# alibaba-damo-academy/Inferix

Hardware: AMD Instinct MI355X
Metric: latent_frames_per_sec (higher is better)
Workload: dtype bf16; 1 GPU; Self-Forcing 480p bf16 (Wan2.1-T2V-1.3B causal DiT, 30 layers), block_size=3, 21 latent frames = 7 blocks x (4 denoise + 1 context) generator forwards, KV prefix 4680..32760 keys in the KV manager's cache (identity page map; page-table form: `streaming_steady`); `value` counts the generator calls (SURVEY 8d), the per-block VAE decode of config 2 is measured beside it under --full (`per_block_decod; batch=1, parallelism=single, layers=30, pair_forwards=True, pair_mode=streams

## Files before the change

include/inferix_hip.h:

```cpp
#ifndef INFERIX_HIP_H
#define INFERIX_HIP_H

#include <stdint.h>

#ifdef __cplusplus
extern "C" {
#endif

#define IFX_OK 0
#define IFX_EINVAL (-1)
#define IFX_ELAUNCH (-2)
#define IFX_EUNSUP (-3)

typedef uint16_t ifx_bf16;

#define IFX_ABI_MINOR 7
int ifx_version(void);
const char* ifx_last_error(void);
const char* ifx_arch(void);
int ifx_set_option(const char* key, int32_t value);
int ifx_get_option(const char* key, int32_t* value);
int32_t ifx_device_error(int32_t clear);

typedef struct {
  ifx_bf16* k;
  ifx_bf16* v;
  const int32_t* page_table;
  int32_t page_size;
  int32_t num_slots;
  int32_t kv_heads;
  int32_t head_dim;
  int32_t seg_split;
  int32_t seg_delta;
} ifx_kv_view;

int ifx_attn_fwd_paged(const ifx_bf16* q, ifx_bf16* out, float* lse, const ifx_kv_view* kv,
                       int32_t q_rows, int32_t heads, int32_t kv_start, int32_t kv_len, float scale,
                       void* stream);

int32_t ifx_attn_split_plan(int32_t q_rows, int32_t heads, int32_t kv_start, int32_t kv_len,
                            int64_t* workspace_bytes);
int ifx_attn_fwd_paged_split(const ifx_bf16* q, ifx_bf16* out, float* lse, const ifx_kv_view* kv,
                             int32_t q_rows, int32_t heads, int32_t kv_start, int32_t kv_len, float scale,
                             int32_t num_splits, void* workspace, int64_t workspace_bytes, void* stream);

int ifx_attn_fwd_paged_ld(const ifx_bf16* q, int32_t ldq, ifx_bf16* out, int32_t ldo, float* lse, const ifx_kv_view* kv,
                          int32_t q_rows, int32_t heads, int32_t kv_start, int32_t kv_len, float scale, int32_t num_splits,
                          void* workspace, int64_t workspace_bytes, void* stream);

int ifx_attn_fwd_dedup(const ifx_bf16* q, ifx_bf16* out, const ifx_kv_view* kv, int32_t q_rows, int32_t heads, int32_t kv_len,
                       int32_t last_key_multiplicity, float scale, void* stream);

int ifx_attn_fwd_ranges(const ifx_bf16* q, int32_t ldq, ifx_bf16* out, int32_t ldo, const ifx_kv_view* kv, int32_t q_rows,
                        int32_t heads, int32_t n_ranges, const int32_t* q_ranges, const int32_t* k_ranges, float scale,
                        void* stream);

int ifx_attn_fwd_partial(const ifx_bf16* q, const ifx_kv_view* kv, int32_t q_rows, int32_t heads, int32_t kv_start,
                         int32_t kv_len, float scale, int32_t num_splits, void* workspace, int64_t workspace_bytes,
                         int32_t slot_base, int32_t slot_cap, int32_t* slots_used, void* stream);
int ifx_attn_merge_partials(const void* workspace, int32_t slot_cap, int32_t slots_used, ifx_bf16* out, float* lse,
                            int32_t q_rows, int32_t heads, void* stream);

int ifx_lse_merge(ifx_bf16* out_a, float* lse_a, const ifx_bf16* out_b, const float* lse_b,
                  int32_t rows, int32_t heads, void* stream);

typedef struct {
  const double* freqs;
  int32_t max_pos;
  int32_t start_frame;
  int32_t height, width;
  int32_t hw_offset;
  int32_t hw_local;
  float q_scale;
  int32_t flags;
} ifx_rope_grid;

int ifx_rmsnorm_rope_kv_append(const ifx_bf16* qkv, int32_t qkv_row_stride, ifx_bf16* q_out,
                               const ifx_bf16* wq, const ifx_bf16* wk, const ifx_rope_grid* rope,
                               const ifx_kv_view* kv, int32_t local_start, int32_t rows,
                               int32_t dim, float eps, void* stream);

int ifx_rmsnorm(const ifx_bf16* x, int32_t x_row_stride, ifx_bf16* y, int32_t y_row_stride,
                const ifx_bf16* w, int32_t rows, int32_t dim, float eps, void* stream);

enum { IFX_LN_PLAIN = 0, IFX_LN_AFFINE = 1, IFX_LN_MODULATE = 2 };
int ifx_layernorm(const ifx_bf16* x, ifx_bf16* y, int32_t rows, int32_t dim, float eps, int32_t mode,
                  const ifx_bf16* gamma, const ifx_bf16* beta, const ifx_bf16* mod,
                  int32_t mod_slots, int32_t shift_slot, int32_t scale_slot, int32_t rows_per_group,
                  void* stream);

enum { IFX_EPI_BIAS = 0, IFX_EPI_GELU_TANH = 1, IFX_EPI_RESIDUAL = 2, IFX_EPI_GATE_RES = 3, IFX_EPI_GELU_ERF = 4 };
typedef struct {
  int32_t epilogue;
  const ifx_bf16* residual;
  int32_t ld_res;
  const ifx_bf16* mod;
  int32_t mod_slots;
  int32_t gate_slot;
  int32_t rows_per_group;
  ifx_bf16* y2;
  int32_t ldy2;
  int32_t split_col;
} ifx_epilogue;
int ifx_gemm_bf16(const ifx_bf16* x, int32_t ldx, const ifx_bf16* w, const ifx_bf16* bias,
                  ifx_bf16* y, int32_t ldy, int32_t M, int32_t N, int32_t K,
                  const ifx_epilogue* epi, void* stream);

int64_t ifx_gemm_workspace_bytes(int32_t M, int32_t N, int32_t K);
int ifx_gemm_bf16_ws(const ifx_bf16* x, int32_t ldx, const ifx_bf16* w, const ifx_bf16* bias, ifx_bf16* y, int32_t ldy,
                     int32_t M, int32_t N, int32_t K, const ifx_epilogue* epi, void* workspace, int64_t workspace_bytes,
                     void* stream);

enum { IFX_Q_FP8_E4M3 = 0, IFX_Q_INT8 = 1 };
int ifx_quant_per_token(const ifx_bf16* x, int32_t ldx, void* q, int32_t ldq, float* scale, int32_t rows,
                        int32_t K, int32_t format, void* stream);
int ifx_gemm_q8(const void* xq, int32_t ldx, const float* x_scale, const void* wq, const float* w_scale,
                const ifx_bf16* bias, ifx_bf16* y, int32_t ldy, int32_t M, int32_t N, int32_t K, int32_t format,
                const ifx_epilogue* epi, void* stream);
int64_t ifx_gemm_q8_workspace_bytes(int32_t M, int32_t N, int32_t K);
int ifx_gemm_q8_ws(const void* xq, int32_t ldx, const float* x_scale, const void* wq, const float* w_scale, const ifx_bf16* bias,
                   ifx_bf16* y, int32_t ldy, int32_t M, int32_t N, int32_t K, int32_t format, const ifx_epilogue* epi,
                   void* workspace, int64_t workspace_bytes, void* stream);
int ifx_layernorm_quant(const ifx_bf16* x, void* q, int32_t ldq, float* scale, int32_t rows, int32_t dim, float eps,
                        int32_t mode, const ifx_bf16* gamma, const ifx_bf16* beta, const ifx_bf16* mod, int32_t mod_slots,
                        int32_t shift_slot, int32_t scale_slot, int32_t rows_per_group, int32_t format, void* stream);

int ifx_gemm_q8_quant_out(const void* xq, int32_t ldx, const float* x_scale, const void* wq, const float* w_scale,
                          const ifx_bf16* bias, void* yq, int32_t ldyq, int32_t M, int32_t N, int32_t K, int32_t format,
                          const ifx_epilogue* epi, const float* out_divisor, int32_t via_bf16, void* stream);
int ifx_layernorm_quant_static(const ifx_bf16* x, void* q, int32_t ldq, const float* divisors, int32_t n_out, int32_t rows,
                               int32_t dim, float eps, int32_t mode, const ifx_bf16* gamma, const ifx_bf16* beta,
                               int32_t via_bf16, void* stream);

int ifx_quant_static(const ifx_bf16* x, int32_t ldx, void* q, int32_t ldq, const float* divisor, int32_t divisor_len,
                     float* row_scale, int32_t rows, int32_t K, int32_t format, int32_t via_bf16, void* stream);
int ifx_quant_per_tensor(const ifx_bf16* x, int32_t ldx, void* q, int32_t ldq, float* row_scale, void* amax_workspace,
                         int32_t rows, int32_t K, int32_t format, void* stream);

int ifx_kv_roll(const ifx_kv_view* kv, int32_t sink_tokens, int32_t evicted, int32_t rolled,
                ifx_bf16* scratch, void* stream);

int ifx_kv_scatter_shards(const ifx_bf16* gathered, int32_t world, int32_t frames, int32_t hw_local,
                          int32_t frame_tokens, int32_t local_start, const ifx_kv_view* kv, void* stream);

#define IFX_MAX_PEERS 8
#define IFX_PEER_HANDLE_BYTES 64
typedef struct {
  int32_t count;
  ifx_bf16* k[IFX_MAX_PEERS];
  ifx_bf16* v[IFX_MAX_PEERS];
} ifx_peer_caches;
typedef struct {
  int32_t count;
  int32_t* flags[IFX_MAX_PEERS];
} ifx_peer_flags;
int ifx_peer_alloc(int64_t bytes, int32_t fine_grained, void** ptr);
int ifx_peer_free(void* ptr);
int ifx_peer_export(const void* ptr, uint8_t* handle, int64_t* offset);
int ifx_peer_open(const uint8_t* handle, void** ptr);
int ifx_peer_close(void* ptr);
int ifx_rmsnorm_rope_kv_push(const ifx_bf16* kv_rows, int32_t kv_row_stride, const ifx_bf16* wk, const ifx_rope_grid* rope,
                             const ifx_peer_caches* peers, const ifx_kv_view* geometry, int32_t local_start, int32_t frame_tokens,
                             int32_t slot_hw_local, int32_t slot_hw_offset, int32_t rows, int32_t dim, float eps, void* stream);
int ifx_peer_signal(const ifx_peer_flags* peers, int32_t index, int32_t value, void* stream);
int ifx_peer_wait(const int32_t* flags, int32_t count, int32_t value, int32_t timeout_ms, int32_t* status, void* stream);

typedef struct {
  const ifx_bf16* x;
  int64_t in_frame_stride;
  const int32_t* in_slots;
  int32_t hs, ws, cin, upsample;
  const ifx_bf16* w;
  const ifx_bf16* bias;
  int32_t kt, ks;
  ifx_bf16* y;
  int64_t out_frame_stride;
  const int32_t* out_slots;
  int32_t cout, t_out;
  const ifx_bf16* residual;
  const void* zero_page;
  int32_t in_planar;
} ifx_conv3d_desc;
int ifx_conv3d_cl(const ifx_conv3d_desc* desc, void* stream);

#define IFX_NORM_SILU 1
#define IFX_NORM_OUT_PLANAR 2
int ifx_rmsnorm_cl(const ifx_bf16* x, const ifx_bf16* gamma, ifx_bf16* y, int64_t out_frame_stride,
                   const int32_t* out_slots, int32_t frames, int32_t frame_pixels, int32_t channels,
                   int32_t flags, void* stream);

int ifx_softmax_rows(const ifx_bf16* scores, ifx_bf16* probs, int32_t rows, int32_t cols, int32_t ld, float scale,
                     void* stream);

int ifx_t5_attention(const ifx_bf16* q, int32_t ldq, const ifx_bf16* k, int32_t ldk, const ifx_bf16* v, int32_t ldv,
                     ifx_bf16* out, int32_t ldo, const ifx_bf16* rel_bias, const int32_t* seq_lens, int32_t batch,
                     int32_t seq_len_padded, int32_t heads, void* stream);

int ifx_t5_gated_gelu(const ifx_bf16* gate_fc1, ifx_bf16* h, int32_t rows, int32_t ffn, void* stream);

typedef struct {
  const ifx_bf16* in;
  int32_t ld_in, rows, layout, q_heads, kv_heads, head_dim;
  const float* rope;
  const float *qn_w, *qn_b, *kn_w, *kn_b;
  const ifx_bf16 *xn_w, *xn_b;
  float eps;
  int32_t layernorm_1p;
  ifx_bf16* q_out;
  int32_t ld_q;
  ifx_bf16* qx_out;
  int32_t ld_qx;
  ifx_bf16* k_out;
  ifx_bf16* v_out;
  int32_t ld_kv, kv_head_stride;
  int32_t row0, split, row1;
  float q_scale;
  int32_t rope_half;
  int32_t q_group;
  int64_t q_group_stride;
} ifx_magi_head_prep_desc;
int ifx_magi_head_prep(const ifx_magi_head_prep_desc* desc, void* stream);

int ifx_magi_gate_norm_residual(const ifx_bf16* x, int32_t ldx, const ifx_bf16* residual, int32_t ld_res,
                                const int32_t* condition_map, const ifx_bf16* gate, int32_t ld_gate, const float* norm_w,
                                const float* norm_b, int32_t layernorm_1p, ifx_bf16* y, int32_t ldy, int32_t rows, int32_t dim,
                                float eps, void* stream);

enum { IFX_ACT_SILU = 0, IFX_ACT_TANH = 1 };
int ifx_act_rows(const ifx_bf16* x, ifx_bf16* y, int64_t n, int32_t mode, void* stream);
int ifx_kv_split_rows(const ifx_bf16* kv, ifx_bf16* k_cache, ifx_bf16* v_cache, int32_t rows, int32_t heads, int32_t row0,
                      int32_t split, int32_t row1, void* stream);

#ifdef __cplusplus
}
#endif
#endif
```

inferix_amd/_hip.py:

```python
from __future__ import annotations

import ctypes as C
import os
from typing import Optional

import torch

_HERE = os.path.dirname(os.path.abspath(__file__))
LIB_PATH = os.environ.get("IFX_HIP_LIB", os.path.join(_HERE, "libinferix_hip.so"))

IFX_LN_PLAIN, IFX_LN_AFFINE, IFX_LN_MODULATE = 0, 1, 2
IFX_EPI_BIAS, IFX_EPI_GELU_TANH, IFX_EPI_RESIDUAL, IFX_EPI_GATE_RES, IFX_EPI_GELU_ERF = 0, 1, 2, 3, 4
IFX_ACT_SILU, IFX_ACT_TANH = 0, 1
IFX_Q_FP8_E4M3, IFX_Q_INT8 = 0, 1


class HipLibraryMissing(RuntimeError):
    pass


class HipKernelError(RuntimeError):
    pass


class KvView(C.Structure):
    _fields_ = [("k", C.c_void_p), ("v", C.c_void_p), ("page_table", C.c_void_p),
                ("page_size", C.c_int32), ("num_slots", C.c_int32), ("kv_heads", C.c_int32),
                ("head_dim", C.c_int32), ("seg_split", C.c_int32), ("seg_delta", C.c_int32)]


class RopeGrid(C.Structure):
    _fields_ = [("freqs", C.c_void_p), ("max_pos", C.c_int32), ("start_frame", C.c_int32),
                ("height", C.c_int32), ("width", C.c_int32), ("hw_offset", C.c_int32),
                ("hw_local", C.c_int32), ("q_scale", C.c_float), ("flags", C.c_int32)]


class Conv3dDesc(C.Structure):
    _fields_ = [("x", C.c_void_p), ("in_frame_stride", C.c_int64), ("in_slots", C.POINTER(C.c_int32)),
                ("hs", C.c_int32), ("ws", C.c_int32), ("cin", C.c_int32), ("upsample", C.c_int32),
                ("w", C.c_void_p), ("bias", C.c_void_p), ("kt", C.c_int32), ("ks", C.c_int32),
                ("y", C.c_void_p), ("out_frame_stride", C.c_int64), ("out_slots", C.POINTER(C.c_int32)),
                ("cout", C.c_int32), ("t_out", C.c_int32), ("residual", C.c_void_p), ("zero_page", C.c_void_p),
                ("in_planar", C.c_int32)]


class Epilogue(C.Structure):
    _fields_ = [("epilogue", C.c_int32), ("residual", C.c_void_p), ("ld_res", C.c_int32),
                ("mod", C.c_void_p), ("mod_slots", C.c_int32), ("gate_slot", C.c_int32),
                ("rows_per_group", C.c_int32), ("y2", C.c_void_p), ("ldy2", C.c_int32), ("split_col", C.c_int32)]


class MagiHeadPrepDesc(C.Structure):
    _fields_ = [("inp", C.c_void_p), ("ld_in", C.c_int32), ("rows", C.c_int32), ("layout", C.c_int32),
                ("q_heads", C.c_int32), ("kv_heads", C.c_int32), ("head_dim", C.c_int32), ("rope", C.c_void_p),
                ("qn_w", C.c_void_p), ("qn_b", C.c_void_p), ("kn_w", C.c_void_p), ("kn_b", C.c_void_p),
                ("xn_w", C.c_void_p), ("xn_b", C.c_void_p), ("eps", C.c_float), ("layernorm_1p", C.c_int32),
                ("q_out", C.c_void_p), ("ld_q", C.c_int32), ("qx_out", C.c_void_p), ("ld_qx", C.c_int32),
                ("k_out", C.c_void_p), ("v_out", C.c_void_p), ("ld_kv", C.c_int32), ("kv_head_stride", C.c_int32),
                ("row0", C.c_int32), ("split", C.c_int32), ("row1", C.c_int32), ("q_scale", C.c_float), ("rope_half", C.c_int32),
                ("q_group", C.c_int32), ("q_group_stride", C.c_int64)]


IFX_MAX_PEERS, IFX_PEER_HANDLE_BYTES = 8, 64


class PeerCaches(C.Structure):
    _fields_ = [("count", C.c_int32), ("k", C.c_void_p * IFX_MAX_PEERS), ("v", C.c_void_p * IFX_MAX_PEERS)]


class PeerFlags(C.Structure):
    _fields_ = [("count", C.c_int32), ("flags", C.c_void_p * IFX_MAX_PEERS)]


_vp, _i32, _f32 = C.c_void_p, C.c_int32, C.c_float
SIGNATURES = {
    "ifx_version": (C.c_int, []),
    "ifx_last_error": (C.c_char_p, []),
    "ifx_arch": (C.c_char_p, []),
    "ifx_set_option": (C.c_int, [C.c_char_p, _i32]),
    "ifx_get_option": (C.c_int, [C.c_char_p, C.POINTER(_i32)]),
    "ifx_device_error": (_i32, [_i32]),
    "ifx_attn_fwd_paged": (C.c_int, [_vp, _vp, _vp, C.POINTER(KvView), _i32, _i32, _i32, _i32, _f32, _vp]),
    "ifx_attn_split_plan": (_i32, [_i32, _i32, _i32, _i32, C.POINTER(C.c_int64)]),
    "ifx_attn_fwd_paged_split": (C.c_int, [_vp, _vp, _vp, C.POINTER(KvView), _i32, _i32, _i32, _i32, _f32, _i32, _vp,
                                           C.c_int64, _vp]),
    "ifx_conv3d_cl": (C.c_int, [C.POINTER(Conv3dDesc), _vp]),
    "ifx_rmsnorm_cl": (C.c_int, [_vp, _vp, _vp, C.c_int64, C.POINTER(_i32), _i32, _i32, _i32, _i32, _vp]),
    "ifx_softmax_rows": (C.c_int, [_vp, _vp, _i32, _i32, _i32, _f32, _vp]),
    "ifx_t5_attention": (C.c_int, [_vp, _i32, _vp, _i32, _vp, _i32, _vp, _i32, _vp, _vp, _i32, _i32, _i32, _vp]),
    "ifx_t5_gated_gelu": (C.c_int, [_vp, _vp, _i32, _i32, _vp]),
    "ifx_kv_scatter_shards": (C.c_int, [_vp, _i32, _i32, _i32, _i32, _i32, C.POINTER(KvView), _vp]),
    "ifx_peer_alloc": (C.c_int, [C.c_int64, _i32, C.POINTER(C.c_void_p)]),
    "ifx_peer_free": (C.c_int, [_vp]),
    "ifx_peer_export": (C.c_int, [_vp, C.c_char_p, C.POINTER(C.c_int64)]),
    "ifx_peer_open": (C.c_int, [C.c_char_p, C.POINTER(C.c_void_p)]),
    "ifx_peer_close": (C.c_int, [_vp]),
    "ifx_rmsnorm_rope_kv_push": (C.c_int, [_vp, _i32, _vp, C.POINTER(RopeGrid), C.POINTER(PeerCaches), C.POINTER(KvView), _i32, _i32,
                                           _i32, _i32, _i32, _i32, _f32, _vp]),
    "ifx_peer_signal": (C.c_int, [C.POINTER(PeerFlags), _i32, _i32, _vp]),
    "ifx_peer_wait": (C.c_int, [_vp, _i32, _i32, _i32, _vp, _vp]),
    "ifx_attn_fwd_partial": (C.c_int, [_vp, C.POINTER(KvView), _i32, _i32, _i32, _i32, _f32, _i32, _vp, C.c_int64, _i32,
                                       _i32, C.POINTER(_i32), _vp]),
    "ifx_attn_merge_partials": (C.c_int, [_vp, _i32, _i32, _vp, _vp, _i32, _i32, _vp]),
    "ifx_lse_merge": (C.c_int, [_vp, _vp, _vp, _vp, _i32, _i32, _vp]),
    "ifx_rmsnorm_rope_kv_append": (C.c_int, [_vp, _i32, _vp, _vp, _vp, C.POINTER(RopeGrid), C.POINTER(KvView),
                                             _i32, _i32, _i32, _f32, _vp]),
    "ifx_rmsnorm": (C.c_int, [_vp, _i32, _vp, _i32, _vp, _i32, _i32, _f32, _vp]),
    "ifx_layernorm": (C.c_int, [_vp, _vp, _i32, _i32, _f32, _i32, _vp, _vp, _vp, _i32, _i32, _i32, _i32, _vp]),
    "ifx_gemm_bf16": (C.c_int, [_vp, _i32, _vp, _vp, _vp, _i32, _i32, _i32, _i32, C.POINTER(Epilogue), _vp]),
    "ifx_kv_roll": (C.c_int, [C.POINTER(KvView), _i32, _i32, _i32, _vp, _vp]),
    "ifx_quant_per_token": (C.c_int, [_vp, _i32, _vp, _i32, _vp, _i32, _i32, _i32, _vp]),
    "ifx_layernorm_quant": (C.c_int, [_vp, _vp, _i32, _vp, _i32, _i32, _f32, _i32, _vp, _vp, _vp, _i32, _i32, _i32, _i32, _i32, _vp]),
    "ifx_gemm_q8": (C.c_int, [_vp, _i32, _vp, _vp, _vp, _vp, _vp, _i32, _i32, _i32, _i32, _i32, C.POINTER(Epilogue), _vp]),
    "ifx_gemm_q8_ws": (C.c_int, [_vp, _i32, _vp, _vp, _vp, _vp, _vp, _i32, _i32, _i32, _i32, _i32, C.POINTER(Epilogue), _vp, C.c_int64, _vp]),
    "ifx_gemm_q8_workspace_bytes": (C.c_int64, [_i32, _i32, _i32]),
    "ifx_attn_fwd_paged_ld": (C.c_int, [_vp, _i32, _vp, _i32, _vp, C.POINTER(KvView), _i32, _i32, _i32, _i32, _f32, _i32, _vp,
                                        C.c_int64, _vp]),
    "ifx_gemm_q8_quant_out": (C.c_int, [_vp, _i32, _vp, _vp, _vp, _vp, _vp, _i32, _i32, _i32, _i32, _i32, C.POINTER(Epilogue), _vp, _i32, _vp]),
    "ifx_layernorm_quant_static": (C.c_int, [_vp, _vp, _i32, _vp, _i32, _i32, _i32, _f32, _i32, _vp, _vp, _i32, _vp]),
    "ifx_quant_static": (C.c_int, [_vp, _i32, _vp, _i32, _vp, _i32, _vp, _i32, _i32, _i32, _i32, _vp]),
    "ifx_quant_per_tensor": (C.c_int, [_vp, _i32, _vp, _i32, _vp, _vp, _i32, _i32, _i32, _vp]),
    "ifx_magi_head_prep": (C.c_int, [C.POINTER(MagiHeadPrepDesc), _vp]),
    "ifx_magi_gate_norm_residual": (C.c_int, [_vp, _i32, _vp, _i32, _vp, _vp, _i32, _vp, _vp, _i32, _vp, _i32, _i32, _i32, _f32,
                                              _vp]),
    "ifx_act_rows": (C.c_int, [_vp, _vp, C.c_int64, _i32, _vp]),
    "ifx_kv_split_rows": (C.c_int, [_vp, _vp, _vp, _i32, _i32, _i32, _i32, _i32, _vp]),
    "ifx_attn_fwd_dedup": (C.c_int, [_vp, _vp, C.POINTER(KvView), _i32, _i32, _i32, _i32, _f32, _vp]),
    "ifx_attn_fwd_ranges": (C.c_int, [_vp, _i32, _vp, _i32, C.POINTER(KvView), _i32, _i32, _i32, C.POINTER(_i32), C.POINTER(_i32), _f32, _vp]),
    "ifx_gemm_workspace_bytes": (C.c_int64, [_i32, _i32, _i32]),
    "ifx_gemm_bf16_ws": (C.c_int, [_vp, _i32, _vp, _vp, _vp, _i32, _i32, _i32, _i32, C.POINTER(Epilogue), _vp, C.c_int64, _vp]),
}

_lib: Optional[C.CDLL] = None
ABI_MINOR = 7


def load() -> C.CDLL:
    global _lib
    if _lib is not None:
        return _lib
    if not os.path.exists(LIB_PATH):
        raise HipLibraryMissing(
            f"{LIB_PATH} not found: build it with `python -c 'import __graft_entry__ as g; g.build()'` "
            "(hipcc --offload-arch=gfx950).  inferix_amd has no CPU or eager fallback.")
    lib = C.CDLL(LIB_PATH)
    for name, (res, args) in SIGNATURES.items():
        fn = getattr(lib, name)
        fn.restype = res
        fn.argtypes = args
    got = (lib.ifx_version() >> 8) & 255
    if got != ABI_MINOR:
        raise HipLibraryMissing(f"{LIB_PATH} has ABI minor {got}, these bindings are for {ABI_MINOR} (include/inferix_hip.h "
                                "IFX_ABI_MINOR): rebuild with __graft_entry__.build()")
    _lib = lib
    return lib


def check(rc: int, what: str) -> None:
    if rc != 0:
        msg = load().ifx_last_error().decode("utf-8", "replace")
        raise HipKernelError(f"{what} failed (code {rc}): {msg}")


def version() -> str:
    v = load().ifx_version()
    return f"{v >> 16}.{(v >> 8) & 255}.{v & 255}"
```

inferix_amd/csrc/ifx_core.hip:

```cpp
#include <stdarg.h>
#include <stdlib.h>
#include <string.h>

#include "ifx_common.h"

namespace ifx {
static thread_local char g_err[512] = "";

void set_error(const char* fmt, ...) {
  va_list ap;
  va_start(ap, fmt);
  vsnprintf(g_err, sizeof(g_err), fmt, ap);
  va_end(ap);
}

static int g_gemm_variant = -1, g_gemm_pp_variant = -1, g_attn_variant = -1, g_conv_variant = -1, g_spin_timeout_ms = -1, g_spin_fault = 0;
static thread_local int g_gemm_small_split = -1;
static int opt_or_env(int& slot, const char* env, int dflt = 0) {
  if (slot < 0) {
    const char* e = getenv(env);
    slot = e ? atoi(e) : dflt;
  }
  return slot;
}
int gemm_variant() { return opt_or_env(g_gemm_variant, "IFX_GEMM_VARIANT"); }
int gemm_pp_variant() { return opt_or_env(g_gemm_pp_variant, "IFX_GEMM_PP_VARIANT"); }
int attn_variant() { return opt_or_env(g_attn_variant, "IFX_ATTN_VARIANT"); }
int conv_variant() { return opt_or_env(g_conv_variant, "IFX_CONV_VARIANT"); }
static unsigned* g_attn_dbg = nullptr;
static bool g_attn_dbg_on = false;
unsigned* attn_debug_counter() { return g_attn_dbg_on ? g_attn_dbg : nullptr; }
int gemm_small_split() { return opt_or_env(g_gemm_small_split, "IFX_GEMM_SMALL_SPLIT"); }

static unsigned* g_dev_err = nullptr;
unsigned* device_error_word() {
  if (g_dev_err == nullptr) {
    void* p = nullptr;
    if (hipHostMalloc(&p, 64, hipHostMallocMapped | hipHostMallocPortable) == hipSuccess && p != nullptr) {
      memset(p, 0, 64);
      g_dev_err = (unsigned*)p;
    }
  }
  return g_dev_err;
}
long long spin_timeout_ticks() { return (long long)max(1, opt_or_env(g_spin_timeout_ms, "IFX_SPIN_TIMEOUT_MS", 2000)) * 100000LL; }
int spin_fault() { return g_spin_fault; }
static thread_local char g_err_dev[640] = "";

int check_launch(const char* what) {
  hipError_t e = hipGetLastError();
  if (e != hipSuccess) {
    set_error("%s: launch failed: %s", what, hipGetErrorString(e));
    return IFX_ELAUNCH;
  }
  return IFX_OK;
}
}

extern "C" int ifx_version(void) { return (0 << 16) | (IFX_ABI_MINOR << 8) | 0; }
extern "C" int32_t ifx_device_error(int32_t clear) {
  unsigned* w = ifx::g_dev_err;
  if (w == nullptr) return 0;
  const unsigned v = __atomic_load_n(w, __ATOMIC_ACQUIRE);
  if (v != 0 && clear) __atomic_store_n(w, 0u, __ATOMIC_RELEASE);
  return (int32_t)v;
}
extern "C" const char* ifx_last_error(void) {
  const unsigned v = (unsigned)ifx_device_error(1);
  if (v == 0) return ifx::g_err;
  const unsigned kind = v >> 24, detail = v & 0xffffffu;
  snprintf(ifx::g_err_dev, sizeof(ifx::g_err_dev),
           "device: a kernel gave up a wait (%s, flag %u) after the spin budget — the producing workgroup was not resident or did not "
           "finish; the results of that launch are invalid%s%s",
           kind == 1 ? "split-K / stream-K consumer of ifx_gemm_bf16_ws / ifx_gemm_q8_ws" : "unknown waiter", detail,
           ifx::g_err[0] ? "; last host error: " : "", ifx::g_err);
  return ifx::g_err_dev;
}
extern "C" const char* ifx_arch(void) { return "gfx950"; }
extern "C" int ifx_set_option(const char* key, int32_t value) {
  if (key && !strcmp(key, "gemm_variant") && value >= 0 && value <= 29) { ifx::g_gemm_variant = value; return IFX_OK; }
  if (key && !strcmp(key, "gemm_small_split") && (value == 0 || value == 1)) { ifx::g_gemm_small_split = value; return IFX_OK; }
  if (key && !strcmp(key, "attn_variant") && value >= 0 && value <= 7) { ifx::g_attn_variant = value; return IFX_OK; }
  if (key && !strcmp(key, "conv_variant") && value >= 0 && value <= 1) { ifx::g_conv_variant = value; return IFX_OK; }
  if (key && !strcmp(key, "gemm_pp_variant") && value >= 0 && value <= 1) { ifx::g_gemm_pp_variant = value; return IFX_OK; }
  if (key && !strcmp(key, "attn_debug_counters") && (value == 0 || value == 1)) {
    if (value == 1) {
      if (ifx::g_attn_dbg == nullptr && hipMalloc((void**)&ifx::g_attn_dbg, 64) != hipSuccess) {
        ifx::g_attn_dbg = nullptr;
        ifx::set_error("ifx_set_option: attn_debug_counters: hipMalloc failed");
        return IFX_ELAUNCH;
      }
      (void)hipDeviceSynchronize();
      (void)hipMemset(ifx::g_attn_dbg, 0, 64);
    }
    ifx::g_attn_dbg_on = value == 1;
    return IFX_OK;
  }
  if (key && !strcmp(key, "spin_timeout_ms") && value >= 1 && value <= 600000) { ifx::g_spin_timeout_ms = value; return IFX_OK; }
  if (key && !strcmp(key, "spin_fault") && (value == 0 || value == 1)) { ifx::g_spin_fault = value; return IFX_OK; }
  ifx::set_error("ifx_set_option: unknown key or value out of range: %s = %d", key ? key : "(null)", (int)value);
  return IFX_EINVAL;
}
extern "C" int ifx_get_option(const char* key, int32_t* value) {
  if (key == nullptr || value == nullptr) { ifx::set_error("ifx_get_option: null argument"); return IFX_EINVAL; }
  if (!strcmp(key, "gemm_variant")) { *value = ifx::gemm_variant(); return IFX_OK; }
  if (!strcmp(key, "gemm_small_split")) { *value = ifx::gemm_small_split(); return IFX_OK; }
  if (!strcmp(key, "attn_variant")) { *value = ifx::attn_variant(); return IFX_OK; }
  if (!strcmp(key, "conv_variant")) { *value = ifx::conv_variant(); return IFX_OK; }
  if (!strcmp(key, "gemm_pp_variant")) { *value = ifx::gemm_pp_variant(); return IFX_OK; }
  if (!strcmp(key, "attn_debug_counters")) { *value = ifx::g_attn_dbg_on ? 1 : 0; return IFX_OK; }
  if (!strcmp(key, "attn_rescale_count")) {
    unsigned v = 0;
    if (ifx::g_attn_dbg != nullptr) {
      (void)hipDeviceSynchronize();
      (void)hipMemcpy(&v, ifx::g_attn_dbg, sizeof(v), hipMemcpyDeviceToHost);
    }
    *value = (int32_t)(v & 0x7fffffffu);
    return IFX_OK;
  }
  if (!strcmp(key, "spin_timeout_ms")) { *value = (int32_t)(ifx::spin_timeout_ticks() / 100000LL); return IFX_OK; }
  if (!strcmp(key, "spin_fault")) { *value = ifx::spin_fault(); return IFX_OK; }
  ifx::set_error("ifx_get_option: unknown key: %s", key);
  return IFX_EINVAL;
}
```

inferix_amd/csrc/ifx_gemm.hip:

```cpp
#include <stdlib.h>

#include "ifx_gemm_epilogue.h"

namespace ifx {

constexpr int BM = 128, BN = 128, BK = 64;

template <int EPI>
__global__ __launch_bounds__(256, 2) void gemm_bf16_kernel(const unsigned short* __restrict__ x, int ldx,
                                                           const unsigned short* __restrict__ w,
                                                           unsigned short* __restrict__ y, int ldy, int M, int N,
                                                           int K, int tiles_m, int tiles_n, EpiArgs ea) {
  extern __shared__ __attribute__((aligned(16))) unsigned char smem[];
  const int tid = threadIdx.x, lane = tid & 63, wave = tid >> 6;
  const int wm = wave & 1, wn = wave >> 1;
  constexpr int GM = 8;
  const int total = tiles_m * tiles_n, per_xcd = (total + 7) / 8;
  const int t_id = (blockIdx.x & 7) * per_xcd + (blockIdx.x >> 3);
  if ((int)(blockIdx.x >> 3) >= per_xcd || t_id >= total) return;
  const int grp_sz = GM * tiles_n;
  const int first_m = (t_id / grp_sz) * GM;
  const int gm = min(GM, tiles_m - first_m);
  const int rem = t_id % grp_sz;
  const int tile_m = first_m + rem % gm, tile_n = rem / gm;
  const int m_base = tile_m * BM, n_base = tile_n * BN;

  const unsigned short* gx[4];
  const unsigned short* gw[4];
  int lds_off[4];
#pragma unroll
  for (int p = 0; p < 4; ++p) {
    const int q = tid + 256 * p, row = q >> 3, c = q & 7;
    const int mr = min(m_base + row, M - 1), nr = min(n_base + row, N - 1);
    gx[p] = x + (size_t)mr * ldx + c * 8;
    gw[p] = w + (size_t)nr * K + c * 8;
    lds_off[p] = row * 128 + ((c ^ (row & 7)) << 4);
  }
  u32x4 rx[4], rw[4];
  auto gload = [&](int kt) {
#pragma unroll
    for (int p = 0; p < 4; ++p) {
      rx[p] = *reinterpret_cast<const u32x4*>(gx[p] + (size_t)kt * BK);
      rw[p] = *reinterpret_cast<const u32x4*>(gw[p] + (size_t)kt * BK);
    }
  };
  auto lstore = [&](int buf) {
    unsigned char* bx = smem + buf * 32768;
    unsigned char* bw = bx + 16384;
#pragma unroll
    for (int p = 0; p < 4; ++p) {
      *reinterpret_cast<u32x4*>(bx + lds_off[p]) = rx[p];
      *reinterpret_cast<u32x4*>(bw + lds_off[p]) = rw[p];
    }
  };

  f32x4 acc[4][4];
#pragma unroll
  for (int i = 0; i < 4; ++i)
#pragma unroll
    for (int j = 0; j < 4; ++j) acc[i][j] = f32x4{0.f, 0.f, 0.f, 0.f};

  const int KT = K / BK;
  gload(0);
  lstore(0);
  __syncthreads();

  const int fr = lane & 15, fq = lane >> 4;
  for (int kt = 0; kt < KT; ++kt) {
    const int buf = kt & 1;
    if (kt + 1 < KT) gload(kt + 1);
    const unsigned char* bx = smem + buf * 32768;
    const unsigned char* bw = bx + 16384;
#pragma unroll
    for (int ks = 0; ks < 2; ++ks) {
      bf16x8 a[4], b[4];
      const int c = ks * 4 + fq;
#pragma unroll
      for (int i = 0; i < 4; ++i) {
        const int row = wn * 64 + i * 16 + fr;
        a[i] = *reinterpret_cast<const bf16x8*>(bw + row * 128 + ((c ^ (row & 7)) << 4));
      }
#pragma unroll
      for (int j = 0; j < 4; ++j) {
        const int row = wm * 64 + j * 16 + fr;
        b[j] = *reinterpret_cast<const bf16x8*>(bx + row * 128 + ((c ^ (row & 7)) << 4));
      }
#pragma unroll
      for (int i = 0; i < 4; ++i)
#pragma unroll
        for (int j = 0; j < 4; ++j)
          acc[i][j] = __builtin_amdgcn_mfma_f32_16x16x32_bf16(a[i], b[j], acc[i][j], 0, 0, 0);
    }
    if (kt + 1 < KT) lstore(buf ^ 1);
    __syncthreads();
  }

#pragma unroll
  for (int j = 0; j < 4; ++j) {
    const int m = m_base + wm * 64 + j * 16 + fr;
    if (m >= M) continue;
    const unsigned short* gate_row = nullptr;
    if (EPI == IFX_EPI_GATE_RES)
      gate_row = ea.mod + ((size_t)(m / ea.rows_per_group) * ea.mod_slots + ea.gate_slot) * N;
#pragma unroll
    for (int i = 0; i < 4; ++i) {
      const int n = n_base + wn * 64 + i * 16 + fq * 4;
      if (n >= N) continue;
      float v[4] = {acc[i][j][0], acc[i][j][1], acc[i][j][2], acc[i][j][3]};
      if (ea.bias) {
        const u16x4 bv = *reinterpret_cast<const u16x4*>(ea.bias + n);
#pragma unroll
        for (int e = 0; e < 4; ++e) v[e] += bf2f(bv[e]);
      }
      u16x4 vb, rv = {}, gv = {};
#pragma unroll
      for (int e = 0; e < 4; ++e) vb[e] = f2bf(v[e]);
      if (EPI == IFX_EPI_RESIDUAL || EPI == IFX_EPI_GATE_RES)
        rv = *reinterpret_cast<const u16x4*>(ea.residual + (size_t)m * ea.ld_res + n);
      if (EPI == IFX_EPI_GATE_RES) gv = *reinterpret_cast<const u16x4*>(gate_row + n);
      const u16x4 o = epi_combine<EPI, 4>(vb, rv, gv, ea.gelu_erf());
      *reinterpret_cast<u16x4*>(y + (size_t)m * ldy + n) = o;
    }
  }
}

static int pick_pp(int M, int N, int K, int mode, bool have_ws) {
  if (N % 64 != 0 || K % 64 != 0) return 0;
  if (have_ws && gemm_pp_split(N, K) && ((M + 255) / 256) * ((N + 255) / 256) <= 1024 && !(gemm_small_split() && M < 2048)) {
    const int tn = (N + 255) / 256, steps = K / 64 / 2;
    const int i4 = ((M + 255) / 256) * tn * 2, i3 = ((M + 191) / 192) * tn * 2;
    const float t4 = ((i4 + 255) / 256) * (steps * 1.6f + 9.f), t3 = ((i3 + 255) / 256) * (steps * 1.4f + 9.f);
    static int allow3 = -1;
    if (allow3 < 0) {
      const char* e = getenv("IFX_PP_SPLIT_TJ3");
      allow3 = e ? atoi(e) : 1;
    }
    return (allow3 && i3 <= 2048 && t3 < t4 && mode != IFX_EPI_GELU_TANH) ? 3 : 4;
  }
  if (M < 1024) return 0;
  static const float step_us[5] = {0.f, 0.f, 1.2f, 1.4f, 1.6f};
  const float tile_us = (mode == IFX_EPI_GELU_TANH ? 8.f : 3.f);
  int best = 0, best_tiles = 0;
  float best_t = 1e30f;
  for (int tj = 4; tj >= 2; --tj) {
    const int tiles = ((M + 64 * tj - 1) / (64 * tj)) * ((N + 255) / 256);
    const int rounds = (tiles + 255) / 256;
    const float t = rounds * ((K / 64) * step_us[tj] + tile_us);
    if (t < best_t) best_t = t, best = tj, best_tiles = tiles;
  }
  if (M < 2048 && best_tiles < 160) return 0;
  return best;
}

static bool want_w4_splitk(int M, int N, int K) {
  const int tiles = ((M + 255) / 256) * ((N + 255) / 256);
  return K >= 4096 && (K / 64) % 2 == 0 && 2 * tiles <= 256 && 2 * tiles >= 160;
}

static int pick_tile(int M, int N, int K) {
  struct Cand { int tile, bm, bn, slots; float base; };
  static const Cand cands[] = {{3, 256, 256, 256, 1.00f}, {19, 256, 192, 256, 0.99f}, {0, 256, 128, 256, 0.85f}, {1, 128, 128, 512, 0.95f},
                               {4, 128, 64, 512, 0.68f},  {2, 64, 64, 512, 0.50f}};
  const int kt = K / 64;
  const int wgs64 = ((M + 63) / 64) * ((N + 63) / 64);
  if (gemm_small_split()) {
    if (wgs64 <= 256 && kt >= 64 && kt % 2 == 0) return 11;
    if (wgs64 <= 256 && kt >= 16 && kt % 4 == 0) return 10;
  }
  const int wgs12864 = ((M + 127) / 128) * ((N + 63) / 64);
  if (wgs12864 > 256 && wgs12864 <= 768) return 13;
  {
    const int t256 = ((M + 255) / 256) * ((N + 255) / 256), rounds = (t256 + 255) / 256;
    if (K >= 2048 && t256 >= 384 && (float)t256 >= 0.7f * 256.f * rounds) return 17;
  }
  int best = 2;
  float best_score = -1.f;
  for (const Cand& c : cands) {
    const int tm = (M + c.bm - 1) / c.bm, tn = (N + c.bn - 1) / c.bn, wgs = tm * tn;
    const int rounds = (wgs + c.slots - 1) / c.slots;
    const float edge = ((float)M * (float)N) / ((float)(tm * c.bm) * (float)(tn * c.bn));
    if (c.tile == 3 && wgs < c.slots && edge < 0.95f) continue;
    const float score = c.base * edge * (float)wgs / (float)(c.slots * rounds);
    if (score > best_score) best_score = score, best = c.tile;
  }
  return best;
}

}

using namespace ifx;

static bool small_split_takes_tile12(int M, int N, int K) {
  if (!gemm_small_split() || N > 2048 || (K / 64) % 2 != 0 || K < 1024) return false;
  const int wgs128 = ((M + 127) / 128) * ((N + 127) / 128);
  return wgs128 > 128 && wgs128 <= 256;
}

static bool small_split_takes_pp_ks4(int M, int N, int K) {
  if (!gemm_small_split() || M >= 2048 || N > 2048 || N % 64 != 0 || K < 4096 || K % 64 != 0 || (K / 64) % 4 != 0) return false;
  const int items = ((M + 127) / 128) * ((N + 255) / 256) * 4;
  return items > 128 && items <= 256;
}

static int gemm_bf16_impl(const ifx_bf16* x, int32_t ldx, const ifx_bf16* w, const ifx_bf16* bias, ifx_bf16* y,
                          int32_t ldy, int32_t M, int32_t N, int32_t K, const ifx_epilogue* epi, void* stream, void* workspace,
                          int64_t workspace_bytes) {
  IFX_REQUIRE(x && w && y && M >= 0 && N > 0 && K > 0, "ifx_gemm_bf16: null/empty operand");
  IFX_REQUIRE(K % BK == 0, "ifx_gemm_bf16: K (%d) must be a multiple of %d", K, BK);
  IFX_REQUIRE(N % 4 == 0 && ldx % 8 == 0 && ldy % 4 == 0, "ifx_gemm_bf16: N %% 4, ldx %% 8, ldy %% 4 required");
  int mode;
  EpiArgsP ea;
  if (const int rc = resolve_epilogue(epi, bias, "ifx_gemm_bf16", &mode, &ea)) return rc;
  if (M == 0) return IFX_OK;
  const int variant = gemm_variant();
  const bool wide_ok = N % 8 == 0 && ldy % 8 == 0 && (ea.residual == nullptr || ea.ld_res % 8 == 0);
  if (wide_ok && variant == 20 && workspace != nullptr && want_w4_splitk(M, N, K) &&
      workspace_bytes >= (int64_t)gemm_w4_workspace_bytes(M, N, 2))
    return launch_gemm_w4(x, ldx, w, y, ldy, M, N, K, mode, ea, (hipStream_t)stream, 2, workspace);
  if (wide_ok && variant == 26 && N % 64 == 0 && K % 64 == 0 && workspace != nullptr &&
      workspace_bytes >= (int64_t)gemm_pp_stream_k_workspace_bytes() && (long)((M + 127) / 128) * ((N + 255) / 256) * (K / 64) >= 48) {
    if (pp_epilogue_fits(mode, ea, 64))
      return launch_gemm_pp(x, ldx, w, y, ldy, M, N, K, mode, ea, (hipStream_t)stream, 2, workspace, 1);
  }
  if (epi != nullptr && epi->y2 != nullptr) {
    IFX_REQUIRE(mode == IFX_EPI_BIAS && wide_ok && N % 64 == 0 && !((uintptr_t)bias & 7) && (variant == 0 || (variant >= 22 && variant <= 25)),
                "ifx_gemm_bf16: the second destination (y2) needs the bias epilogue, N %% 64 == 0, 8-byte aligned bias and the ping-pong tiles");
    int tj = variant == 0 ? pick_pp(M, N, K, mode, false) : (variant == 22 || variant == 25 ? 4 : variant == 23 ? 3 : 2);
    if (tj == 0) tj = 2;
    ea.y2 = epi->y2, ea.ldy2 = epi->ldy2, ea.split_col = epi->split_col;
    return launch_gemm_pp(x, ldx, w, y, ldy, M, N, K, mode, ea, (hipStream_t)stream, tj, nullptr);
  }
  if (wide_ok && variant >= 27 && variant <= 29) {
    const int ks = 2 << (variant - 27);
    const bool fits = N % 64 == 0 && K % 64 == 0 && (K / 64) % ks == 0 && workspace != nullptr &&
                      workspace_bytes >= (int64_t)gemm_pp_small_workspace_bytes(M, N, ks) &&
                      (long)((M + 127) / 128) * ((N + 255) / 256) * (ks - 1) <= 1024 && pp_epilogue_fits(mode, ea, 64);
    if (fits)
      return launch_gemm_pp(x, ldx, w, y, ldy, M, N, K, mode, ea, (hipStream_t)stream, 2, workspace, 0, 0, ks);
  }
  if (wide_ok && variant == 0 && small_split_takes_pp_ks4(M, N, K) && workspace != nullptr &&
      workspace_bytes >= (int64_t)gemm_pp_small_workspace_bytes(M, N, 4)) {
    if (pp_epilogue_fits(mode, ea, 64))
      return launch_gemm_pp(x, ldx, w, y, ldy, M, N, K, mode, ea, (hipStream_t)stream, 2, workspace, 0, 0, 4);
  }
  if (wide_ok && variant == 0 && small_split_takes_tile12(M, N, K))
    return launch_gemm_lds_dma(12, x, ldx, w, y, ldy, M, N, K, mode, ea, (hipStream_t)stream);
  if (wide_ok && (variant == 0 || (variant >= 22 && variant <= 25))) {
    const bool ws_ok = workspace != nullptr && workspace_bytes >= (int64_t)gemm_pp_workspace_bytes(M, N, K) && variant != 25;
    int tj = variant == 0 ? pick_pp(M, N, K, mode, ws_ok) : (variant == 22 || variant == 25 ? 4 : variant == 23 ? 3 : 2);
    const bool fits = N % 64 == 0 && pp_epilogue_fits(mode, ea, 32 * tj);
    if (tj && (fits || variant != 0))
      return launch_gemm_pp(x, ldx, w, y, ldy, M, N, K, mode, ea, (hipStream_t)stream, tj, ws_ok ? workspace : nullptr);
  }
  if (wide_ok && variant != 1) {
    const int tile = (variant >= 2 && variant != 20 && variant != 26) ? variant - 2 : pick_tile(M, N, K);
    return launch_gemm_lds_dma(tile, x, ldx, w, y, ldy, M, N, K, mode, ea, (hipStream_t)stream);
  }
  const int tiles_m = (M + BM - 1) / BM, tiles_n = (N + BN - 1) / BN;
  const dim3 grid(((tiles_m * tiles_n + 7) / 8) * 8), block(256);
  const size_t lds = 65536;
  hipStream_t s = (hipStream_t)stream;
  const int rc = dispatch_epilogue(mode, "ifx_gemm_bf16", [&](auto epi_c) {
    constexpr int E = decltype(epi_c)::value;
    static bool attr_set = false;
    if (!attr_set) {
      (void)hipFuncSetAttribute((const void*)gemm_bf16_kernel<E>, hipFuncAttributeMaxDynamicSharedMemorySize, (int)lds);
      attr_set = true;
    }
    hipLaunchKernelGGL((gemm_bf16_kernel<E>), grid, block, lds, s, x, ldx, w, y, ldy, M, N, K, tiles_m, tiles_n, ea);
  });
  if (rc != IFX_OK) return rc;
  return check_launch("ifx_gemm_bf16");
}

extern "C" int ifx_gemm_bf16(const ifx_bf16* x, int32_t ldx, const ifx_bf16* w, const ifx_bf16* bias, ifx_bf16* y,
                             int32_t ldy, int32_t M, int32_t N, int32_t K, const ifx_epilogue* epi, void* stream) {
  return gemm_bf16_impl(x, ldx, w, bias, y, ldy, M, N, K, epi, stream, nullptr, 0);
}

extern "C" int64_t ifx_gemm_workspace_bytes(int32_t M, int32_t N, int32_t K) {
  if (M <= 0 || N <= 0 || K <= 0) return 0;
  const int v = gemm_variant();
  if (v == 20) return want_w4_splitk(M, N, K) ? (int64_t)gemm_w4_workspace_bytes(M, N, 2) : 0;
  if (v == 26 && N % 64 == 0 && K % 64 == 0) return (int64_t)gemm_pp_stream_k_workspace_bytes();
  if (v >= 27 && v <= 29) return (N % 64 == 0 && K % 64 == 0 && (K / 64) % (2 << (v - 27)) == 0) ? (int64_t)gemm_pp_small_workspace_bytes(M, N, 2 << (v - 27)) : 0;
  if (v == 0 && small_split_takes_pp_ks4(M, N, K)) return (int64_t)gemm_pp_small_workspace_bytes(M, N, 4);
  if (v == 0 && N % 8 == 0 && small_split_takes_tile12(M, N, K)) return 0;
  if ((v == 0 && N % 64 == 0 && K % 64 == 0 && !(gemm_small_split() && M < 2048)) || v == 22) return (int64_t)gemm_pp_workspace_bytes(M, N, K);
  return 0;
}

extern "C" int ifx_gemm_bf16_ws(const ifx_bf16* x, int32_t ldx, const ifx_bf16* w, const ifx_bf16* bias, ifx_bf16* y,
                                int32_t ldy, int32_t M, int32_t N, int32_t K, const ifx_epilogue* epi, void* workspace,
                                int64_t workspace_bytes, void* stream) {
  return gemm_bf16_impl(x, ldx, w, bias, y, ldy, M, N, K, epi, stream, workspace, workspace_bytes);
}
```

inferix_amd/csrc/ifx_gemm_epilogue.h:

```cpp
#pragma once
#include <type_traits>

#include "ifx_common.h"

namespace ifx {

struct EpiArgs {
  const unsigned short* bias = nullptr;
  const unsigned short* residual = nullptr;
  int ld_res = 0;
  const unsigned short* mod = nullptr;
  int mod_slots = 1, gate_slot = 0, rows_per_group = 1;
  __host__ __device__ bool gelu_erf() const { return gate_slot != 0; }
};

struct EpiArgsQ : EpiArgs {
  const float* sa = nullptr;
  const float* sw = nullptr;
  const float* qdiv = nullptr;
  int q_via_bf16 = 0;
};

struct EpiArgsP : EpiArgsQ {
  unsigned short* y2 = nullptr;
  int ldy2 = 0, split_col = 0;
};

template <int W>
using u16v = unsigned short __attribute__((ext_vector_type(W)));

template <int EPI, int W>
__device__ __forceinline__ u16v<W> epi_combine(const u16v<W> vv, const u16v<W> rv, const u16v<W> gv, const bool erf) {
  u16v<W> o;
  if constexpr (EPI == IFX_EPI_BIAS) {
    o = vv;
  } else if constexpr (EPI == IFX_EPI_GELU_TANH) {
    if (erf) {
#pragma unroll
      for (int e = 0; e < W; ++e) o[e] = f2bf(gelu_erf_f(bf2f(vv[e])));
    } else {
#pragma unroll
      for (int e = 0; e < W; ++e) o[e] = f2bf(gelu_tanh_fast(bf2f(vv[e])));
    }
  } else if constexpr (EPI == IFX_EPI_RESIDUAL) {
#pragma unroll
    for (int e = 0; e < W; ++e) o[e] = f2bf(bf2f(rv[e]) + bf2f(vv[e]));
  } else {
    static_assert(EPI == IFX_EPI_GATE_RES, "epilogue");
#pragma unroll
    for (int e = 0; e < W; ++e) o[e] = f2bf(bf2f(rv[e]) + rbf(bf2f(vv[e]) * bf2f(gv[e])));
  }
  return o;
}

template <int EPI, int W>
__device__ __forceinline__ u16v<W> epi_apply(const u16v<W> vv, int m, int n, int N, const EpiArgs& ea) {
  u16v<W> rv = vv, gv = vv;
  if constexpr (EPI == IFX_EPI_RESIDUAL || EPI == IFX_EPI_GATE_RES)
    rv = *reinterpret_cast<const u16v<W>*>(ea.residual + (size_t)m * ea.ld_res + n);
  if constexpr (EPI == IFX_EPI_GATE_RES)
    gv = *reinterpret_cast<const u16v<W>*>(ea.mod + ((size_t)(m / ea.rows_per_group) * ea.mod_slots + ea.gate_slot) * N + n);
  return epi_combine<EPI, W>(vv, rv, gv, ea.gelu_erf());
}

template <int EPI>
__device__ __forceinline__ void epi_store_row(const u16x8 vv, int m, int n, int N, const EpiArgs& ea, unsigned short* __restrict__ y,
                                              int ldy) {
  *reinterpret_cast<u16x8*>(y + (size_t)m * ldy + n) = epi_apply<EPI, 8>(vv, m, n, N, ea);
}


template <typename F>
static inline int dispatch_epilogue(int mode, const char* what, F&& launch) {
  switch (mode) {
    case IFX_EPI_BIAS: launch(std::integral_constant<int, IFX_EPI_BIAS>{}); return IFX_OK;
    case IFX_EPI_GELU_TANH: launch(std::integral_constant<int, IFX_EPI_GELU_TANH>{}); return IFX_OK;
    case IFX_EPI_RESIDUAL: launch(std::integral_constant<int, IFX_EPI_RESIDUAL>{}); return IFX_OK;
    case IFX_EPI_GATE_RES: launch(std::integral_constant<int, IFX_EPI_GATE_RES>{}); return IFX_OK;
    default: set_error("%s: unknown epilogue %d", what, mode); return IFX_EINVAL;
  }
}

static inline int resolve_epilogue(const ifx_epilogue* epi, const unsigned short* bias, const char* who, int* mode, EpiArgs* ea) {
  *mode = epi ? epi->epilogue : IFX_EPI_BIAS;
  *ea = EpiArgs{};
  ea->bias = bias;
  if (*mode == IFX_EPI_GELU_ERF) {
    *mode = IFX_EPI_GELU_TANH;
    ea->gate_slot = 1;
  }
  if (*mode == IFX_EPI_RESIDUAL || *mode == IFX_EPI_GATE_RES) {
    IFX_REQUIRE(epi->residual && epi->ld_res % 4 == 0, "%s: residual epilogue needs residual/ld_res", who);
    ea->residual = epi->residual;
    ea->ld_res = epi->ld_res;
  }
  if (*mode == IFX_EPI_GATE_RES) {
    IFX_REQUIRE(epi->mod && epi->rows_per_group > 0 && epi->gate_slot >= 0 && epi->gate_slot < epi->mod_slots,
                "%s: gate epilogue needs mod/mod_slots/gate_slot/rows_per_group", who);
    ea->mod = epi->mod;
    ea->mod_slots = epi->mod_slots;
    ea->gate_slot = epi->gate_slot;
    ea->rows_per_group = epi->rows_per_group;
  }
  return IFX_OK;
}

static inline bool pp_epilogue_fits(int mode, const EpiArgs& ea, int min_rows_per_group) {
  const bool res = mode == IFX_EPI_RESIDUAL || mode == IFX_EPI_GATE_RES;
  return !((uintptr_t)ea.bias & 7) && (!res || (!((uintptr_t)ea.residual & 15) && ea.ld_res % 8 == 0)) &&
         (mode != IFX_EPI_GATE_RES || (!((uintptr_t)ea.mod & 15) && ea.rows_per_group >= min_rows_per_group));
}

int launch_gemm_lds_dma(int tile, const unsigned short* x, int ldx, const unsigned short* w, unsigned short* y, int ldy, int M, int N,
                        int K, int mode, const EpiArgs& ea, hipStream_t s);
int launch_gemm_glds(const unsigned short* x, int ldx, const unsigned short* w, unsigned short* y, int ldy, int M, int N, int K,
                     int mode, const EpiArgs& ea, hipStream_t s);
int launch_gemm_w4(const unsigned short* x, int ldx, const unsigned short* w, unsigned short* y, int ldy, int M, int N, int K,
                   int mode, const EpiArgs& ea, hipStream_t s, int splits, void* workspace);
size_t gemm_w4_workspace_bytes(int M, int N, int splits);
int launch_gemm_pp(const unsigned short* x, int ldx, const unsigned short* w, unsigned short* y, int ldy, int M, int N, int K,
                   int mode, const EpiArgsP& ea, hipStream_t s, int tj, void* workspace, int stream_k = 0, int q8_int8 = 0,
                   int force_ks = 0);
size_t gemm_pp_small_workspace_bytes(int M, int N, int ks);
size_t gemm_pp_stream_k_workspace_bytes();
bool gemm_pp_split(int N, int K);
size_t gemm_pp_workspace_bytes(int M, int N, int K);

}
```

inferix_amd/csrc/ifx_gemm_pp.hip:

```cpp
#include <stdlib.h>

#include "ifx_gemm_epilogue.h"

#ifndef IFX_PP_TRACE
#define IFX_PP_TRACE 0
#endif
#ifndef IFX_PP_LAB
#define IFX_PP_LAB IFX_PP_TRACE
#endif


namespace ifx {

namespace gpp {
constexpr int BN = 256, BK = 64;
constexpr int SLOT = 16384, STAGE = 4 * SLOT, SCRATCH = 2 * STAGE;
constexpr int LDS_BYTES = SCRATCH + 32768;
constexpr int X_UP = 0, W_LO = SLOT, W_HI = 2 * SLOT, X_DN = 3 * SLOT;
constexpr int LX_STAGE = 16384, LX_DN = 8192, LW_BASE = 32768, LW_STAGE = 32768;
typedef int v4i __attribute__((ext_vector_type(4)));
typedef int v8i __attribute__((ext_vector_type(8)));
typedef int v16i __attribute__((ext_vector_type(16)));
typedef __attribute__((address_space(3))) void* lds_ptr_t;

__device__ __forceinline__ void dma16(v4i rsrc, unsigned lds, int voff, int soff) {
  asm volatile("s_mov_b32 m0, %0\n\ts_nop 0\n\tbuffer_load_dwordx4 %1, %2, %3 offen lds"
               :
               : "s"(lds), "v"(voff), "s"(rsrc), "s"(soff)
               : "memory");
}
__device__ __forceinline__ v4i make_rsrc(const void* base, unsigned num_bytes) {
  const unsigned long long a = (unsigned long long)base;
  v4i r;
  r[0] = (int)(unsigned)a;
  r[1] = (int)((unsigned)(a >> 32) & 0xffffu);
  r[2] = (int)num_bytes;
  r[3] = 0x00020000;
  return r;
}
template <int N>
__device__ __forceinline__ void wait_vm() {
  asm volatile("s_waitcnt vmcnt(%0)" ::"n"(N) : "memory");
}
template <int N, bool ON>
__device__ __forceinline__ void wait_vm_if() {
  if constexpr (ON) wait_vm<N>();
}
__device__ __forceinline__ void wait_lds() { __builtin_amdgcn_s_waitcnt(0xC07F); }

struct Cursor {
  int i, kt, g, rot, k0, len;
  int kb;
  unsigned stg;
  v4i rs;
};
}

template <int EPI, int TJ, int KS, int Q8 = 0, int LW = 0>
__global__ __launch_bounds__(LW ? 768 : 512, LW ? 3 : 2) void gemm_pp_kernel(const unsigned short* __restrict__ x, int ldx,
                                                         const unsigned short* __restrict__ w, unsigned short* __restrict__ y,
                                                         int ldy, int M, int N, int K, int tiles_m, int total, int per_xcd,
                                                         int wg_per_xcd, EpiArgsP ea, unsigned long long* __restrict__ trace, int dbg,
                                                         float* __restrict__ ws_part, unsigned* __restrict__ ws_flag,
                                                         unsigned* __restrict__ err_word, long long spin_ticks) {
  using namespace gpp;
  static_assert(!LW || (TJ == 2 && KS == 1 && Q8 == 0), "the loader-wave form is the unsplit bf16 128-token tile");
  dbg = IFX_PP_LAB ? dbg : (dbg & 32);
  constexpr int BM = 64 * TJ;
  constexpr int GM = 4;
  constexpr bool RES = EPI == IFX_EPI_RESIDUAL || EPI == IFX_EPI_GATE_RES;
  extern __shared__ __attribute__((aligned(16))) unsigned char smem[];
  const int tid = threadIdx.x, lane = tid & 63;
  const int wave = __builtin_amdgcn_readfirstlane(tid >> 6);
  const int grp = wave >> 2, w4 = wave & 3;
  constexpr int ES = Q8 ? 1 : 2;
  const unsigned char* const xb = reinterpret_cast<const unsigned char*>(x);
  const unsigned char* const wb = reinterpret_cast<const unsigned char*>(w);
  constexpr bool SK = KS == 0;
  constexpr int KSD = KS > 0 ? KS : 1;
  const int S = K * ES / 128;
  const int KT = S / KSD;
  const int tiles_n = total / KSD / tiles_m;

  const int xcd = blockIdx.x & 7, slot_i = blockIdx.x >> 3;
  const int id_first = xcd * per_xcd + slot_i;
  const int id_end = min(xcd * per_xcd + per_xcd, total);
  if (!SK && id_first >= id_end) return;
  const int sk_P = (int)gridDim.x, sk_p = xcd * (sk_P >> 3) + slot_i;
  auto sk_start = [&](int q) __attribute__((always_inline)) { return (int)((long)q * total * S / sk_P); };
  const int sk_u0 = SK ? sk_start(sk_p) : 0, sk_u1 = SK ? sk_start(sk_p + 1) : 0;
  const int sk_t0 = SK ? sk_u0 / S : 0;
  const int n_my = SK ? (sk_u1 - 1) / S - sk_t0 + 1 : (id_end - id_first + wg_per_xcd - 1) / wg_per_xcd;
  const int G = SK ? sk_u1 - sk_u0 : n_my * KT;
  auto item_split = [&](int i) __attribute__((always_inline)) { return KS > 1 ? (id_first + i * wg_per_xcd) % KSD : 0; };
  auto item_tile = [&](int i) __attribute__((always_inline)) { return SK ? sk_t0 + i : (id_first + i * wg_per_xcd) / KSD; };
  auto item_k0 = [&](int i) __attribute__((always_inline)) { return SK ? (i == 0 ? sk_u0 - sk_t0 * S : 0) : item_split(i) * KT; };
  auto item_len = [&](int i) __attribute__((always_inline)) {
    return SK ? min(S, sk_u1 - (sk_t0 + i) * S) - (i == 0 ? sk_u0 - sk_t0 * S : 0) : KT;
  };
  auto item_dumps = [&](int i) __attribute__((always_inline)) { return SK ? (i == 0 && sk_u0 > sk_t0 * S) : (KS > 1 && item_split(i) >= 1); };
  auto item_parts = [&](int i) __attribute__((always_inline)) {
    if (!SK) return KS > 1 ? KS - 1 : 0;
    const int t_end = (sk_t0 + i + 1) * S;
    int n = 0;
    while (sk_p + 1 + n < sk_P && sk_start(sk_p + 1 + n) < t_end) ++n;
    return sk_u1 < t_end ? n : 0;
  };
  auto tile_base = [&](int i, int& m_base, int& n_base) __attribute__((always_inline)) {
    const int t_id = item_tile(i);
    const int grp_sz = GM * tiles_n;
    const int first_m = (t_id / grp_sz) * GM;
    const int gm = min(GM, tiles_m - first_m);
    const int rem = t_id % grp_sz;
    m_base = (first_m + rem % gm) * BM;
    n_base = (rem / gm) * BN;
  };

  const int r8 = lane >> 3, pc = lane & 7;
  const int prow = w4 * 8 + r8;
  const int ld_op = grp == 0 ? K : ldx;
  const int voff = prow * ld_op * ES + ((pc ^ ((prow >> 1) & 7)) << 4);
  const int voff_w = LW ? prow * K * ES + ((pc ^ ((prow >> 1) & 7)) << 4) : 0;
  const int voff_x = LW ? prow * ldx * ES + ((pc ^ ((prow >> 1) & 7)) << 4) : 0;
  const unsigned lds_piece0 = (unsigned)(unsigned long long)(lds_ptr_t)smem + w4 * 1024;
  auto cur_desc = [&](Cursor& c, bool is_w) __attribute__((always_inline)) {
    int mb, nb;
    tile_base(c.i, mb, nb);
    if (dbg & 1) mb = nb = 0;
    c.rot = (!SK && (dbg & 4)) ? ((nb / BN) * 3) % KT : 0;
    c.k0 = item_k0(c.i);
    c.len = item_len(c.i);
    c.kb = c.k0 * 128;
    if (is_w) c.rs = make_rsrc(wb + (size_t)nb * K * ES, (unsigned)min(((long)N - nb) * (long)K * ES, 0xffffffffL));
    else c.rs = make_rsrc(xb + (size_t)mb * ldx * ES, (unsigned)min(((long)M - mb - 1) * (long)ldx * ES + (long)K * ES, 0xffffffffL));
  };
  auto cur_init = [&](Cursor& c, bool is_w) __attribute__((always_inline)) {
    c.i = 0, c.kt = 0, c.g = 0, c.stg = 0;
    cur_desc(c, is_w);
  };
  auto cur_next = [&](Cursor& c, bool is_w) __attribute__((always_inline)) {
    ++c.g;
    if constexpr (LW) c.stg = !is_w ? c.stg ^ LX_STAGE : c.stg == 2 * LW_STAGE ? 0 : c.stg + LW_STAGE;
    else c.stg ^= STAGE;
    c.kb += 128;
    if (++c.kt == c.len) {
      c.kt = 0;
      if (++c.i < n_my) cur_desc(c, is_w);
    }
  };
  auto issue = [&](const Cursor& c, bool is_w, int slot, int row0, int pieces) __attribute__((always_inline)) {
    const int kk = c.kt + c.rot;
    const int kb = IFX_PP_LAB ? ((!SK && kk >= KT ? kk - KT : kk) + c.k0) * 128 : c.kb;
    const unsigned p = lds_piece0 + c.stg + slot;
    if ((dbg & 8) && c.g >= 2) return;
    const int vo = LW ? (is_w ? voff_w : voff_x) : voff;
    const int pitch = LW ? (is_w ? K : ldx) : ld_op;
#pragma unroll
    for (int q = 0; q < 4; ++q)
      if (q < pieces) dma16(c.rs, p + q * 4096, vo, kb + (row0 + q * 32) * pitch * ES);
  };
  const bool opw = grp == 0;
  auto req_w = [&](Cursor& c) __attribute__((always_inline)) {
    if constexpr (!LW) issue(c, opw, W_LO, 0, 4), issue(c, opw, W_HI, 128, 4), cur_next(c, opw);
  };
  auto req_x = [&](Cursor& c, int slot, int row0) __attribute__((always_inline)) {
    if constexpr (!LW) issue(c, opw, slot, row0, TJ), cur_next(c, opw);
  };
  Cursor ca, cb;
  cur_init(ca, opw);
  cur_init(cb, opw);

  constexpr bool MF16 = Q8 == 0;
  const int l31 = lane & 31, hi = lane >> 5, l15 = lane & 15, q4 = lane >> 4;
  int lane_ks[4];
#pragma unroll
  for (int ks = 0; ks < 4; ++ks)
    lane_ks[ks] = MF16 ? l15 * 128 + ((((4 * ks + q4) & 7) ^ ((l15 >> 1) & 7)) << 4)
                       : l31 * 128 + (((2 * ks + hi) ^ ((l31 >> 1) & 7)) << 4);
  const int w_frag_off = (w4 >> 1) * SLOT + (w4 & 1) * 8192 + W_LO;
  const int x_frag_off = grp == 0 ? X_UP : X_DN;
  bf16x8 fx[4][TJ], fw[4][2], fx16[2 * TJ][2];
  int rg = 0;
  int rw = 0;
  const int w_off_lw = (w4 >> 1) * SLOT + (w4 & 1) * 8192, x_off_lw = grp == 0 ? 0 : LX_DN;
  auto read_frags = [&]() __attribute__((always_inline)) {
    const unsigned char* st = smem + (rg & 1) * STAGE;
    const unsigned char* const wst = LW ? smem + LW_BASE + rw * LW_STAGE + w_off_lw : st + w_frag_off;
    const unsigned char* const xst = LW ? smem + (rg & 1) * LX_STAGE + x_off_lw : st + x_frag_off;
    if constexpr (LW) rw = rw == 2 ? 0 : rw + 1;
    if constexpr (MF16) {
#pragma unroll
      for (int kk = 0; kk < 2; ++kk) {
#pragma unroll
        for (int c = 0; c < 4; ++c) fw[c][kk] = *reinterpret_cast<const bf16x8*>(wst + lane_ks[kk] + c * 2048);
#pragma unroll
        for (int t = 0; t < 2 * TJ; ++t) fx16[t][kk] = *reinterpret_cast<const bf16x8*>(xst + lane_ks[kk] + t * 2048);
      }
    } else {
#pragma unroll
      for (int ks = 0; ks < 4; ++ks) {
#pragma unroll
        for (int i = 0; i < 2; ++i) fw[ks][i] = *reinterpret_cast<const bf16x8*>(st + w_frag_off + lane_ks[ks] + i * 4096);
#pragma unroll
        for (int j = 0; j < TJ; ++j) fx[ks][j] = *reinterpret_cast<const bf16x8*>(st + x_frag_off + lane_ks[ks] + j * 4096);
      }
    }
    ++rg;
  };

  f32x16 acc[2][TJ];
  f32x4 acc16[4][2 * TJ];
  auto quad = [&](int i, int j, int g) __attribute__((always_inline)) {
    if constexpr (MF16) return acc16[g][2 * j + i];
    else return f32x4{acc[i][j][4 * g], acc[i][j][4 * g + 1], acc[i][j][4 * g + 2], acc[i][j][4 * g + 3]};
  };
  auto mfma16 = [&](bool first) __attribute__((always_inline)) {
    const f32x4 z = {0.f, 0.f, 0.f, 0.f};
#pragma unroll
    for (int kk = 0; kk < 2; ++kk)
#pragma unroll
      for (int c = 0; c < 4; ++c)
#pragma unroll
        for (int t = 0; t < 2 * TJ; ++t)
          acc16[c][t] = __builtin_amdgcn_mfma_f32_16x16x32_bf16(fw[c][kk], fx16[t][kk], first && kk == 0 ? z : acc16[c][t], 0, 0, 0);
  };
  auto q8_mfma = [&](int kk, int i, int j, const f32x16 c) __attribute__((always_inline)) {
    const v8i a = __builtin_shufflevector(__builtin_bit_cast(v4i, fw[2 * kk][i]), __builtin_bit_cast(v4i, fw[2 * kk + 1][i]), 0, 1, 2, 3, 4, 5, 6, 7);
    const v8i b = __builtin_shufflevector(__builtin_bit_cast(v4i, fx[2 * kk][j]), __builtin_bit_cast(v4i, fx[2 * kk + 1][j]), 0, 1, 2, 3, 4, 5, 6, 7);
    return __builtin_amdgcn_mfma_scale_f32_32x32x64_f8f6f4(a, b, c, 0, 0, 0, 0x7f7f7f7f, 0, 0x7f7f7f7f);
  };
  auto i8_mfma = [&](int ks, int i, int j, const f32x16 c) __attribute__((always_inline)) {
    return __builtin_bit_cast(f32x16, __builtin_amdgcn_mfma_i32_32x32x32_i8(__builtin_bit_cast(v4i, fw[ks][i]), __builtin_bit_cast(v4i, fx[ks][j]),
                                                                            __builtin_bit_cast(v16i, c), 0, 0, 0));
  };
  auto mfma_first = [&]() __attribute__((always_inline)) {
    const f32x16 z = {0.f, 0.f, 0.f, 0.f, 0.f, 0.f, 0.f, 0.f, 0.f, 0.f, 0.f, 0.f, 0.f, 0.f, 0.f, 0.f};
    if constexpr (Q8 == 2) {
#pragma unroll
      for (int ks = 0; ks < 4; ++ks)
#pragma unroll
        for (int i = 0; i < 2; ++i)
#pragma unroll
          for (int j = 0; j < TJ; ++j) acc[i][j] = i8_mfma(ks, i, j, ks == 0 ? z : acc[i][j]);
      return;
    }
    if constexpr (Q8 == 1) {
#pragma unroll
      for (int i = 0; i < 2; ++i)
#pragma unroll
        for (int j = 0; j < TJ; ++j) acc[i][j] = q8_mfma(0, i, j, z);
#pragma unroll
      for (int i = 0; i < 2; ++i)
#pragma unroll
        for (int j = 0; j < TJ; ++j) acc[i][j] = q8_mfma(1, i, j, acc[i][j]);
      return;
    }
    mfma16(true);
  };
  auto mfma_next = [&]() __attribute__((always_inline)) {
    if constexpr (Q8 == 2) {
#pragma unroll
      for (int ks = 0; ks < 4; ++ks)
#pragma unroll
        for (int i = 0; i < 2; ++i)
#pragma unroll
          for (int j = 0; j < TJ; ++j) acc[i][j] = i8_mfma(ks, i, j, acc[i][j]);
      return;
    }
    if constexpr (Q8 == 1) {
#pragma unroll
      for (int kk = 0; kk < 2; ++kk)
#pragma unroll
        for (int i = 0; i < 2; ++i)
#pragma unroll
          for (int j = 0; j < TJ; ++j) acc[i][j] = q8_mfma(kk, i, j, acc[i][j]);
      return;
    }
    mfma16(false);
  };

  unsigned char* const tw = smem + SCRATCH + wave * 4096;
  const __amdgpu_buffer_rsrc_t rs_ws =
      __builtin_amdgcn_make_buffer_rsrc((void*)ws_part, 0,
                                        KS != 1 ? (int)min((long)(SK ? sk_P : total / KSD * (KSD - 1)) * BM * BN * 4L, 0x7fffffffL) : 0, 0x00020000);
  auto part_slot = [&](int i) __attribute__((always_inline)) {
    return SK ? sk_p : item_tile(i) * (KSD - 1) + (item_split(i) > 0 ? item_split(i) - 1 : 0);
  };
  auto part_soff = [&](int i) __attribute__((always_inline)) { return part_slot(i) * (BM * BN * 4) + wave * (TJ * 8192); };
  auto flag_of = [&](int i) __attribute__((always_inline)) { return part_slot(i); };
  auto dump_partial = [&](int i) __attribute__((always_inline)) {
    int ln = __builtin_amdgcn_mbcnt_hi(~0u, __builtin_amdgcn_mbcnt_lo(~0u, 0u));
    asm volatile("" : "+v"(ln));
    const int so = part_soff(i);
#pragma unroll
    for (int ii = 0; ii < 2; ++ii)
#pragma unroll
      for (int j = 0; j < TJ; ++j)
#pragma unroll
        for (int q = 0; q < 4; ++q) {
          const f32x4 v = quad(ii, j, q);
          __builtin_amdgcn_raw_buffer_store_b128(__builtin_bit_cast(u32x4, v), rs_ws, ln * 16 + ((ii * TJ + j) * 4 + q) * 1024, so, 16);
        }
  };
  int flag_pending = 0;
  auto consumer_sync = [&](int i) __attribute__((always_inline)) {
    const int first = SK ? sk_p + 1 : item_tile(i) * (KSD - 1), n = item_parts(i);
    if (wave == 0) {
      const long long t0 = wall_clock64();
      bool gave_up = false;
      for (int q = 0; q < n && !gave_up; ++q)
        while (__hip_atomic_load(ws_flag + first + q, __ATOMIC_RELAXED, __HIP_MEMORY_SCOPE_AGENT) == 0u) {
          __builtin_amdgcn_s_sleep(4);
          if (wall_clock64() - t0 > spin_ticks) {
            gave_up = true;
            if (err_word != nullptr)
              __hip_atomic_store(err_word, (1u << 24) | ((unsigned)(first + q) & 0xffffffu), __ATOMIC_RELAXED, __HIP_MEMORY_SCOPE_SYSTEM);
            break;
          }
        }
    }
    __builtin_amdgcn_s_barrier();
    asm volatile("" ::: "memory");
    if (wave == 0)
      for (int q = 0; q < n; ++q) __hip_atomic_store(ws_flag + first + q, 0u, __ATOMIC_RELAXED, __HIP_MEMORY_SCOPE_AGENT);
  };
  auto epilogue = [&](int i_tile, auto between) __attribute__((always_inline)) {
    between();
    int ln = __builtin_amdgcn_mbcnt_hi(~0u, __builtin_amdgcn_mbcnt_lo(~0u, 0u));
    asm volatile("" : "+v"(ln));
    const int l31 = ln & 31, hi = ln >> 5, rr = ln >> 3, cc = ln & 7;
    auto quad_ch = [&](int i, int g) __attribute__((always_inline)) { return MF16 ? g * 16 + (ln >> 4) * 4 : i * 32 + g * 8 + hi * 4; };
    int m_base, n_base;
    tile_base(i_tile, m_base, n_base);
    const int part_so = KS != 1 ? part_soff(i_tile) + (SK ? BM * BN * 4 : 0) : 0;
    const int part_n = KS != 1 ? item_parts(i_tile) : 0;
    const int e_n0 = min(n_base + w4 * 64, N - 64);
    const bool n_ok = n_base + w4 * 64 < N;
    const int e_m0 = m_base + grp * (32 * TJ);
    const bool has_bias = ea.bias != nullptr;
    const unsigned short* const bias_p = has_bias ? ea.bias : y;
    const unsigned bias_mask = has_bias ? 0xffffffffu : 0u;
    constexpr bool PRIV = Q8 != 0 && RES && TJ == 4;
    u32x2 e_bias[2][4];
    int q_bias[2] = {0, 0}, q_sw[4] = {0, 0, 0, 0};
    if constexpr (PRIV) {
      const u32x2 b = *reinterpret_cast<const u32x2*>(bias_p + e_n0 + (ln & 7) * 8 + hi * 4);
      q_bias[0] = (int)(b[0] & bias_mask), q_bias[1] = (int)(b[1] & bias_mask);
      const u32x4 sq = *reinterpret_cast<const u32x4*>(ea.sw + e_n0 + (ln & 7) * 8 + hi * 4);
#pragma unroll
      for (int e = 0; e < 4; ++e) q_sw[e] = (int)sq[e];
    } else {
#pragma unroll
      for (int i = 0; i < (MF16 ? 1 : 2); ++i)
#pragma unroll
        for (int g = 0; g < 4; ++g) {
          const u32x2 b = *reinterpret_cast<const u32x2*>(bias_p + e_n0 + quad_ch(i, g));
          e_bias[i][g] = u32x2{b[0] & bias_mask, b[1] & bias_mask};
        }
    }
    f32x4 e_sw[Q8 ? 2 : 1][Q8 ? 4 : 1];
    float e_sa[Q8 ? TJ : 1];
    f32x4 e_qd[2];
    if constexpr (Q8) {
      if constexpr (!PRIV) {
#pragma unroll
        for (int i = 0; i < 2; ++i)
#pragma unroll
          for (int g = 0; g < 4; ++g) e_sw[i][g] = *reinterpret_cast<const f32x4*>(ea.sw + e_n0 + i * 32 + g * 8 + hi * 4);
      }
#pragma unroll
      for (int j = 0; j < TJ; ++j) e_sa[j] = ea.sa[min(e_m0 + j * 32 + l31, M - 1)];
      if constexpr (EPI == IFX_EPI_GELU_TANH) {
        const float* const qd = ea.qdiv != nullptr ? ea.qdiv : ea.sw;
        e_qd[0] = *reinterpret_cast<const f32x4*>(qd + e_n0 + cc * 8);
        e_qd[1] = *reinterpret_cast<const f32x4*>(qd + e_n0 + cc * 8 + 4);
      }
    }
    u32x4 e_res[2][4], e_gate[2];
    int e_split = 0;
    auto fetch_res = [&](int j) __attribute__((always_inline)) {
      if constexpr (RES) {
#pragma unroll
        for (int p = 0; p < 4; ++p) {
          const int m = min(e_m0 + j * 32 + p * 8 + rr, M - 1);
          e_res[j & 1][p] = *reinterpret_cast<const u32x4*>(ea.residual + (size_t)m * ea.ld_res + e_n0 + cc * 8);
        }
      }
    };
    if constexpr (RES) {
      fetch_res(0);
      if constexpr (EPI == IFX_EPI_GATE_RES) {
        const int m_hi = min(e_m0 + 32 * TJ - 1, M - 1);
        const int g_lo = min(e_m0, M - 1) / ea.rows_per_group, g_hi = m_hi / ea.rows_per_group;
        e_split = (g_lo + 1) * ea.rows_per_group;
        e_gate[0] = *reinterpret_cast<const u32x4*>(ea.mod + ((size_t)g_lo * ea.mod_slots + ea.gate_slot) * N + e_n0 + cc * 8);
        e_gate[1] = *reinterpret_cast<const u32x4*>(ea.mod + ((size_t)g_hi * ea.mod_slots + ea.gate_slot) * N + e_n0 + cc * 8);
      }
    }
    unsigned char* const wr = MF16 ? tw + (ln & 15) * 128 + ((ln >> 4) & 1) * 8 : tw + l31 * 128 + hi * 8;
    const unsigned char* const rd = tw + rr * 128;
    const bool to_y2 = ea.y2 != nullptr && e_n0 >= ea.split_col;
    const int ldo = to_y2 ? ea.ldy2 : ldy;
    unsigned short* const yrow = (to_y2 ? ea.y2 - ea.split_col : y) + (size_t)(e_m0 + rr) * ldo + e_n0 + cc * 8;
    if constexpr (PRIV) {
      asm volatile("" : "+v"(q_bias[0]), "+v"(q_bias[1]), "+v"(q_sw[0]), "+v"(q_sw[1]), "+v"(q_sw[2]), "+v"(q_sw[3]));
    } else {
#pragma unroll
      for (int i = 0; i < (MF16 ? 1 : 2); ++i)
#pragma unroll
        for (int g = 0; g < 4; ++g) asm volatile("" : "+v"(e_bias[i][g]));
    }
    if constexpr (Q8) {
      if constexpr (!PRIV) {
#pragma unroll
        for (int i = 0; i < 2; ++i)
#pragma unroll
          for (int g = 0; g < 4; ++g) asm volatile("" : "+v"(e_sw[i][g]));
      }
#pragma unroll
      for (int j = 0; j < TJ; ++j) asm volatile("" : "+v"(e_sa[j]));
      if constexpr (EPI == IFX_EPI_GELU_TANH) asm volatile("" : "+v"(e_qd[0]), "+v"(e_qd[1]));
    }
#pragma unroll
    for (int j = 0; j < TJ; ++j) {
      if (j + 1 < TJ) fetch_res(j + 1);
#pragma unroll
      for (int i = 0; i < 2; ++i) {
#pragma unroll
        for (int g = 0; g < 4; ++g) {
          const f32x4 aq = quad(i, j, g);
          float v[4] = {aq[0], aq[1], aq[2], aq[3]};
          if constexpr (Q8 == 2 && KS <= 1) {
#pragma unroll
            for (int e = 0; e < 4; ++e) v[e] = (float)__builtin_bit_cast(int, v[e]);
          }
          if constexpr (KS > 1) {
            f32x4 pq[KSD - 1];
#pragma unroll
            for (int q = 0; q < KSD - 1; ++q)
              pq[q] = __builtin_bit_cast(f32x4, __builtin_amdgcn_raw_buffer_load_b128(rs_ws, ln * 16 + ((i * TJ + j) * 4 + g) * 1024,
                                                                                      part_so + q * (BM * BN * 4), 16));
            if constexpr (Q8 == 2) {
              int vi[4];
#pragma unroll
              for (int e = 0; e < 4; ++e) vi[e] = __builtin_bit_cast(int, v[e]);
#pragma unroll
              for (int q = 0; q < KSD - 1; ++q)
#pragma unroll
                for (int e = 0; e < 4; ++e) {
                  const float pe = pq[q][e];
                  vi[e] += __builtin_bit_cast(int, pe);
                }
#pragma unroll
              for (int e = 0; e < 4; ++e) v[e] = (float)vi[e];
            } else {
#pragma unroll
              for (int q = 0; q < KSD - 1; ++q)
#pragma unroll
                for (int e = 0; e < 4; ++e) v[e] += pq[q][e];
            }
          }
          if constexpr (SK) {
            for (int q = 0; q < part_n; ++q) {
              const f32x4 pq = __builtin_bit_cast(f32x4, __builtin_amdgcn_raw_buffer_load_b128(
                                                             rs_ws, ln * 16 + ((i * TJ + j) * 4 + g) * 1024, part_so + q * (BM * BN * 4), 16));
#pragma unroll
              for (int e = 0; e < 4; ++e) v[e] += pq[e];
            }
          }
          if constexpr (Q8) {
            f32x4 swv;
            if constexpr (PRIV) {
#pragma unroll
              for (int e = 0; e < 4; ++e)
                swv[e] = __builtin_bit_cast(float, __builtin_amdgcn_ds_bpermute(((ln & 32) | (i * 4 + g)) << 2, q_sw[e]));
            } else {
              swv = e_sw[i][g];
            }
#pragma unroll
            for (int e = 0; e < 4; ++e) v[e] = __fmul_rn(v[e], __fmul_rn(e_sa[j], swv[e]));
          }
          u32x2 b;
          if constexpr (PRIV) {
            b[0] = (unsigned)__builtin_amdgcn_ds_bpermute(((ln & 32) | (i * 4 + g)) << 2, q_bias[0]);
            b[1] = (unsigned)__builtin_amdgcn_ds_bpermute(((ln & 32) | (i * 4 + g)) << 2, q_bias[1]);
          } else {
            b = e_bias[MF16 ? 0 : i][g];
          }
          v[0] += __builtin_bit_cast(float, b[0] << 16);
          v[1] += __builtin_bit_cast(float, b[0] & 0xffff0000u);
          v[2] += __builtin_bit_cast(float, b[1] << 16);
          v[3] += __builtin_bit_cast(float, b[1] & 0xffff0000u);
          u16x4 o;
#pragma unroll
          for (int e = 0; e < 4; ++e) o[e] = f2bf(v[e]);
          if constexpr (MF16) *reinterpret_cast<u16x4*>(wr + i * 2048 + (((2 * g + hi) ^ cc) << 4)) = o;
          else *reinterpret_cast<u16x4*>(wr + (((i * 4 + g) ^ (l31 & 7)) << 4)) = o;
        }
      }
      wait_lds();
#pragma unroll
      for (int p = 0; p < 4; ++p) {
        const int mrow = p * 8 + rr;
        const int m = e_m0 + j * 32 + mrow;
        const u16x8 vv = *reinterpret_cast<const u16x8*>(rd + p * 1024 + ((cc ^ (mrow & 7)) << 4));
        if constexpr (RES) asm volatile("" : "+v"(e_res[j & 1][p]));
        if constexpr (EPI == IFX_EPI_GATE_RES) {
          if (j == 0 && p == 0) asm volatile("" : "+v"(e_gate[0]), "+v"(e_gate[1]));
        }
        u16x8 o;
        if constexpr (EPI == IFX_EPI_GELU_TANH) {
          if (ea.gelu_erf()) {
#pragma unroll
            for (int e = 0; e < 8; ++e) o[e] = f2bf(gelu_erf_f(bf2f(vv[e])));
          } else {
#pragma unroll
            for (int e = 0; e < 8; ++e) o[e] = f2bf(gelu_tanh_fast(bf2f(vv[e])));
          }
        } else {
          u16x8 rv = vv, gv = vv;
          if constexpr (RES) rv = __builtin_bit_cast(u16x8, e_res[j & 1][p]);
          if constexpr (EPI == IFX_EPI_GATE_RES) gv = __builtin_bit_cast(u16x8, m >= e_split ? e_gate[1] : e_gate[0]);
          o = epi_combine<EPI, 8>(vv, rv, gv, false);
        }
        if constexpr (Q8 && EPI == IFX_EPI_GELU_TANH) {
          if (ea.qdiv != nullptr) {
            unsigned wq[2];
#pragma unroll
            for (int h = 0; h < 2; ++h) {
              float t[4];
#pragma unroll
              for (int e = 0; e < 4; ++e) {
                const float q = fminf(fmaxf(bf2f(o[4 * h + e]) / e_qd[h][e], -448.0f), 448.0f);
                t[e] = ea.q_via_bf16 ? rbf(q) : q;
              }
              unsigned pk = __builtin_amdgcn_cvt_pk_fp8_f32(t[0], t[1], 0u, false);
              wq[h] = __builtin_amdgcn_cvt_pk_fp8_f32(t[2], t[3], pk, true);
            }
            if (m < M && n_ok)
              *reinterpret_cast<u32x2*>(reinterpret_cast<unsigned char*>(y) + (size_t)(e_m0 + rr + j * 32 + p * 8) * ldy + e_n0 + cc * 8) =
                  u32x2{wq[0], wq[1]};
            continue;
          }
        }
        if (m < M && n_ok) *reinterpret_cast<u16x8*>(yrow + (size_t)(j * 32 + p * 8) * ldo) = o;
      }
    }
  };

#if IFX_PP_TRACE
  unsigned long long seg[6] = {0, 0, 0, 0, 0, 0};
  unsigned long long t_last = __builtin_readcyclecounter();
  int seg_i = 0;
#define PP_STAMP()                                                 \
  do {                                                             \
    const unsigned long long t_now = __builtin_readcyclecounter(); \
    seg[seg_i] += t_now - t_last;                                  \
    t_last = t_now;                                                \
    seg_i = seg_i == 5 ? 0 : seg_i + 1;                            \
  } while (0)
#else
#define PP_STAMP() \
  do {             \
  } while (0)
#endif
#ifndef IFX_PP_STAGGER
#define IFX_PP_STAGGER 0
#endif
  auto roles = [&](auto stagger_tag) __attribute__((always_inline)) {
  constexpr bool reads_first = decltype(stagger_tag)::value;

  int kt = 0, it = 0;
  int klen = item_len(0);
  if (grp == 0) {
    req_w(ca);
    wait_vm_if<0, !LW>();
    __builtin_amdgcn_s_barrier();
    for (int g = 0; g < G; ++g) {
      PP_STAMP();
      const bool epi = g > 0 && kt == 0;
      const bool issued = ca.g < G;
      const bool early_reads = reads_first && !epi;
      if (epi && KS != 1 && item_dumps(it - 1)) {
        if (issued) req_w(ca);
        PP_STAMP();
        dump_partial(it - 1);
        wait_vm<0>();
        flag_pending = flag_of(it - 1) + 1;
        PP_STAMP();
        read_frags();
      } else if (epi) {
        if (KS != 1) consumer_sync(it - 1);
        epilogue(it - 1, [&]() __attribute__((always_inline)) {
          if (issued) req_w(ca);
          PP_STAMP();
        });
        PP_STAMP();
        read_frags();
      } else if (early_reads) {
        read_frags();
        if (issued) req_w(ca);
        PP_STAMP();
        PP_STAMP();
      } else {
        if (issued) req_w(ca);
        PP_STAMP();
        PP_STAMP();
        read_frags();
      }
      wait_lds();
      __builtin_amdgcn_sched_barrier(0);
      PP_STAMP();
      __builtin_amdgcn_s_barrier();
      __builtin_amdgcn_sched_barrier(0);
      PP_STAMP();
      if (KS != 1 && flag_pending) {
        if (wave == 0 && !(dbg & 32)) __hip_atomic_store(ws_flag + flag_pending - 1, 1u, __ATOMIC_RELAXED, __HIP_MEMORY_SCOPE_AGENT);
        flag_pending = 0;
      }
      if (!(dbg & 2)) {
        if (kt == 0) mfma_first();
        else mfma_next();
      }
      if (++kt == klen) kt = 0, ++it, klen = it < n_my ? item_len(it) : 0;
      wait_vm_if<0, !LW>();
      __builtin_amdgcn_sched_barrier(0);
      PP_STAMP();
      __builtin_amdgcn_s_barrier();
      __builtin_amdgcn_sched_barrier(0);
    }
    if (KS != 1 && item_dumps(it - 1)) {
      dump_partial(it - 1);
      wait_vm<0>();
      flag_pending = flag_of(it - 1) + 1;
    } else {
      if (KS != 1) consumer_sync(it - 1);
      epilogue(it - 1, [&]() __attribute__((always_inline)) {});
    }
    if (KS != 1) {
      __builtin_amdgcn_s_barrier();
      if (flag_pending && wave == 0 && !(dbg & 32)) __hip_atomic_store(ws_flag + flag_pending - 1, 1u, __ATOMIC_RELAXED, __HIP_MEMORY_SCOPE_AGENT);
    }
  } else {
    req_x(cb, X_UP, 0);
    req_x(ca, X_DN, 32 * TJ);
    if (cb.g < G) req_x(cb, X_UP, 0);
    if (G > 1) wait_vm_if<2 * TJ, !LW>();
    else wait_vm_if<TJ, !LW>();
    __builtin_amdgcn_s_barrier();
    if (G > 1) wait_vm_if<TJ, !LW>();
    else wait_vm_if<0, !LW>();
    __builtin_amdgcn_s_barrier();
    for (int g = 0; g < G; ++g) {
      PP_STAMP();
      const bool lower = ca.g < G, upper = cb.g < G;
      if (reads_first) {
        read_frags();
        if (lower) req_x(ca, X_DN, 32 * TJ);
        if (upper) req_x(cb, X_UP, 0);
        PP_STAMP();
        PP_STAMP();
      } else {
        if (lower) req_x(ca, X_DN, 32 * TJ);
        if (upper) req_x(cb, X_UP, 0);
        PP_STAMP();
        PP_STAMP();
        read_frags();
      }
      wait_lds();
      if (upper) wait_vm_if<2 * TJ, !LW>();
      else if (lower) wait_vm_if<TJ, !LW>();
      else wait_vm_if<0, !LW>();
      __builtin_amdgcn_sched_barrier(0);
      PP_STAMP();
      __builtin_amdgcn_s_barrier();
      __builtin_amdgcn_sched_barrier(0);
      PP_STAMP();
      if (!(dbg & 2)) {
        if (kt == 0) mfma_first();
        else mfma_next();
      }
      if (++kt == klen) kt = 0, ++it, klen = it < n_my ? item_len(it) : 0;
      if (upper) wait_vm_if<TJ, !LW>();
      else wait_vm_if<0, !LW>();
      __builtin_amdgcn_sched_barrier(0);
      PP_STAMP();
      if (kt == 0) {
        if (KS != 1 && item_dumps(it - 1)) {
          dump_partial(it - 1);
          wait_vm<0>();
        } else {
          if (KS != 1) consumer_sync(it - 1);
          epilogue(it - 1, [&]() __attribute__((always_inline)) {});
        }
      }
      if (g + 1 < G || KS != 1) {
        __builtin_amdgcn_s_barrier();
        __builtin_amdgcn_sched_barrier(0);
      }
    }
  }
  };
  auto loader = [&]() __attribute__((always_inline)) {
    Cursor cw, cu, cl;
    cur_init(cw, true), cur_init(cu, false), cur_init(cl, false);
    auto w_step = [&]() __attribute__((always_inline)) {
      issue(cw, true, LW_BASE, 0, 4), issue(cw, true, LW_BASE + SLOT, 128, 4), cur_next(cw, true);
    };
    auto up_step = [&]() __attribute__((always_inline)) { issue(cu, false, 0, 0, TJ), cur_next(cu, false); };
    auto lo_step = [&]() __attribute__((always_inline)) { issue(cl, false, LX_DN, 32 * TJ, TJ), cur_next(cl, false); };
    w_step(), up_step();
    if (G > 1) w_step();
    lo_step();
    if (G > 1) up_step(), wait_vm<8 + 2 * TJ>();
    else wait_vm<TJ>();
    __builtin_amdgcn_s_barrier();
    __builtin_amdgcn_sched_barrier(0);
#if IFX_PP_TRACE
    t_last = __builtin_readcyclecounter();
#endif
    for (int g = 0; g < G; ++g) {
      const bool more = g + 1 < G, more2 = g + 2 < G;
      if (more2) w_step();
      PP_STAMP();
      if (more2) wait_vm<TJ + 8>();
      else if (more) wait_vm<TJ>();
      else wait_vm<0>();
      __builtin_amdgcn_sched_barrier(0);
      PP_STAMP();
      __builtin_amdgcn_s_barrier();
      __builtin_amdgcn_sched_barrier(0);
      PP_STAMP();
      if (more) lo_step();
      if (more2) up_step();
      PP_STAMP();
      if (more2) wait_vm<8 + 2 * TJ>();
      else if (more) wait_vm<TJ>();
      else wait_vm<0>();
      __builtin_amdgcn_sched_barrier(0);
      PP_STAMP();
      __builtin_amdgcn_s_barrier();
      __builtin_amdgcn_sched_barrier(0);
      PP_STAMP();
    }
  };
  if (LW && grp == 2) loader();
  else if (IFX_PP_STAGGER && (w4 & 1)) roles(std::true_type{});
  else roles(std::false_type{});
#if IFX_PP_TRACE
  if (trace != nullptr && blockIdx.x == 0 && lane == 0 && (wave & 3) == 0) {
#pragma unroll
    for (int k = 0; k < 6; ++k) trace[grp * 8 + k] = seg[k];
    trace[grp * 8 + 6] = (unsigned long long)G;
  }
#endif
}

bool gemm_pp_split(int N, int K) {
  static int min_k = -1;
  if (min_k < 0) {
    const char* e = getenv("IFX_PP_SPLIT_MIN_K");
    min_k = e ? atoi(e) : 4096;
  }
  return K >= min_k && N <= 2048 && (K / 64) % 2 == 0;
}
size_t gemm_pp_stream_k_workspace_bytes() { return 4096 + (size_t)256 * 128 * 256 * 4; }
size_t gemm_pp_workspace_bytes(int M, int N, int K) {
  if (!gemm_pp_split(N, K)) return 0;
  const size_t tn = (size_t)(N + 255) / 256;
  const size_t t4 = (size_t)((M + 255) / 256) * tn, t3 = (size_t)((M + 191) / 192) * tn;
  if (t4 > 1024) return 0;
  const size_t b4 = t4 * 256 * 256 * 4, b3 = t3 <= 1024 ? t3 * 192 * 256 * 4 : 0;
  return 4096 + (b4 > b3 ? b4 : b3);
}

size_t gemm_pp_small_workspace_bytes(int M, int N, int ks) {
  if (ks <= 1) return 0;
  const size_t tiles = (size_t)((M + 127) / 128) * ((N + 255) / 256);
  return 4096 + tiles * (size_t)(ks - 1) * 128 * 256 * 4;
}

int launch_gemm_pp(const unsigned short* x, int ldx, const unsigned short* w, unsigned short* y, int ldy, int M, int N, int K,
                   int mode, const EpiArgsP& ea, hipStream_t s, int tj, void* workspace, int stream_k, int q8_int8, int force_ks) {
  using namespace gpp;
  const bool q8 = ea.sa != nullptr;
  if (ea.y2 != nullptr && (q8 || ea.split_col <= 0 || ea.split_col % BN != 0 || ea.split_col >= N || ea.ldy2 % 8 != 0 || ((uintptr_t)ea.y2 & 15))) {
    set_error("ifx_gemm_bf16: the second destination needs bf16 operands, 0 < split_col < N a multiple of %d, ldy2 %% 8 == 0 and a 16-byte aligned y2", BN);
    return IFX_EINVAL;
  }
  if (q8 && (K % 128 != 0 || ldx % 16 != 0 || ((uintptr_t)ea.sw & 15) || ((uintptr_t)ea.qdiv & 15))) {
    set_error("ifx_gemm_q8: the ping-pong tile needs K %% 128 == 0, ldx %% 16 == 0 and 16-byte aligned scale vectors (K = %d, ldx = %d)", K, ldx);
    return IFX_EINVAL;
  }
  if (N % 64 != 0 || K % 64 != 0) {
    set_error("ifx_gemm_bf16: the ping-pong tile needs N and K to be multiples of 64 (N = %d, K = %d)", N, K);
    return IFX_EINVAL;
  }
  if (mode == IFX_EPI_GATE_RES && ea.rows_per_group < 32 * tj) {
    set_error("ifx_gemm_bf16: the ping-pong tile needs gate groups of at least %d rows (rows_per_group = %d)", 32 * tj, ea.rows_per_group);
    return IFX_EINVAL;
  }
  if (!pp_epilogue_fits(mode, ea, 0)) {
    set_error("ifx_gemm_bf16: the ping-pong tile needs 8-byte aligned bias and 16-byte aligned residual / gate rows");
    return IFX_EINVAL;
  }
  static int cu_of_dev[16] = {0};
  int dev = 0, n_cu = 0;
  if (hipGetDevice(&dev) == hipSuccess && dev >= 0 && dev < 16) {
    if (cu_of_dev[dev] == 0) {
      int v = 0;
      cu_of_dev[dev] = hipDeviceGetAttribute(&v, hipDeviceAttributeMultiprocessorCount, dev) == hipSuccess && v > 0 ? v : 256;
    }
    n_cu = cu_of_dev[dev];
  }
  if (n_cu <= 0) n_cu = 256;
  const int BM = 64 * tj;
  const int tiles_m = (M + BM - 1) / BM, tiles_n = (N + BN - 1) / BN;
  int ks = stream_k ? 0 : ((tj == 4 || (tj == 3 && !q8)) && workspace != nullptr && gemm_pp_split(N, q8 ? K / 2 : K) &&
                           tiles_m * tiles_n <= 1024) ? 2 : 1;
  if (force_ks > 1) {
    if (q8 || stream_k || tj != 2 || workspace == nullptr || (K / 64) % force_ks != 0 || tiles_m * tiles_n * (force_ks - 1) > 1024 ||
        (force_ks != 2 && force_ks != 4 && force_ks != 8)) {
      set_error("ifx_gemm_bf16: the %d-way K split needs the bf16 128-token tile, a workspace, K / 64 divisible by it and at most 1024 partial slots",
                force_ks);
      return IFX_EINVAL;
    }
    ks = force_ks;
  }
  const int total = tiles_m * tiles_n * (ks ? ks : 1), per_xcd = (total + 7) / 8;
  int wg_per_xcd = min(per_xcd, max(1, n_cu / 8));
  if (stream_k) {
    const long units = (long)total * (K * (q8 ? 1 : 2) / 128);
    if (q8 || tj != 2 || workspace == nullptr || units < 8) {
      set_error("ifx_gemm_bf16: stream-K needs the bf16 128-token tile, a workspace and at least 8 K-steps");
      return IFX_EINVAL;
    }
    wg_per_xcd = (int)max(1L, min((long)min(n_cu, 256) / 8, units / 6 / 8));
  }
  const dim3 grid(wg_per_xcd * 8);
  unsigned* ws_flag = (unsigned*)workspace;
  float* ws_part = workspace ? (float*)((char*)workspace + 4096) : nullptr;
  static unsigned long long* trace = nullptr;
  static int dbg = -1;
  if (dbg < 0) {
    const char* e = getenv("IFX_PP_DEBUG");
    dbg = e ? atoi(e) : 0;
  }
  const int dbg_launch = dbg | (spin_fault() ? 32 : 0);
  unsigned* const err_word = device_error_word();
  const long long spin_ticks = spin_timeout_ticks();
#if IFX_PP_TRACE
  if (!trace) {
    const char* e = getenv("IFX_PP_TRACE_PTR");
    if (e) trace = (unsigned long long*)strtoull(e, nullptr, 0);
  }
#endif
#define IFX_LAUNCH_PP(E, T, S, Q, L)                                                                                                 \
  do {                                                                                                                               \
    static bool attr_set = false;                                                                                                    \
    if (!attr_set) {                                                                                                                 \
      (void)hipFuncSetAttribute((const void*)gemm_pp_kernel<E, T, S, Q, L>, hipFuncAttributeMaxDynamicSharedMemorySize, (int)LDS_BYTES); \
      attr_set = true;                                                                                                               \
    }                                                                                                                                \
    hipLaunchKernelGGL((gemm_pp_kernel<E, T, S, Q, L>), grid, dim3(L ? 768 : 512), LDS_BYTES, s, x, ldx, w, y, ldy, M, N, K, tiles_m, \
                       total, per_xcd, wg_per_xcd, ea, trace, dbg_launch, ws_part, ws_flag, err_word, spin_ticks);                   \
  } while (0)
#define IFX_SWITCH_PP_L(T, S, Q, L)                                                                             \
  {                                                                                                             \
    const int rc = dispatch_epilogue(mode, "ifx_gemm(pp)", [&](auto epi_c) { IFX_LAUNCH_PP(decltype(epi_c)::value, T, S, Q, L); }); \
    if (rc != IFX_OK) return rc;                                                                                \
  }
#define IFX_SWITCH_PP(T, S, Q) IFX_SWITCH_PP_L(T, S, Q, 0)
  if (q8 && ks == 2) {
    if (q8_int8) { IFX_SWITCH_PP(4, 2, 2) }
    else { IFX_SWITCH_PP(4, 2, 1) }
  } else if (q8 && q8_int8) {
    if (tj == 4) { IFX_SWITCH_PP(4, 1, 2) }
    else if (tj == 3) { IFX_SWITCH_PP(3, 1, 2) }
    else if (tj == 2) { IFX_SWITCH_PP(2, 1, 2) }
    else { set_error("ifx_gemm_q8: no ping-pong tile of %d tokens", 64 * tj); return IFX_EINVAL; }
  } else if (q8) {
    if (tj == 4) { IFX_SWITCH_PP(4, 1, 1) }
    else if (tj == 3) { IFX_SWITCH_PP(3, 1, 1) }
    else if (tj == 2) { IFX_SWITCH_PP(2, 1, 1) }
    else { set_error("ifx_gemm_q8: no ping-pong tile of %d tokens", 64 * tj); return IFX_EINVAL; }
  } else if (ks == 0) {
    IFX_SWITCH_PP(2, 0, 0)
  } else if (tj == 2 && ks == 2) { IFX_SWITCH_PP(2, 2, 0)
  } else if (tj == 2 && ks == 4) { IFX_SWITCH_PP(2, 4, 0)
  } else if (tj == 2 && ks == 8) { IFX_SWITCH_PP(2, 8, 0)
  } else if (ks == 2) {
    if (tj == 4) { IFX_SWITCH_PP(4, 2, 0) }
    else { IFX_SWITCH_PP(3, 2, 0) }
  } else if (tj == 4) { IFX_SWITCH_PP(4, 1, 0) }
  else if (tj == 3) { IFX_SWITCH_PP(3, 1, 0) }
  else if (tj == 2 && gemm_pp_variant() == 1) { IFX_SWITCH_PP(2, 1, 0) }
  else if (tj == 2) { IFX_SWITCH_PP_L(2, 1, 0, 1) }
  else { set_error("ifx_gemm_bf16: no ping-pong tile of %d tokens", 64 * tj); return IFX_EINVAL; }
#undef IFX_SWITCH_PP
#undef IFX_SWITCH_PP_L
#undef IFX_LAUNCH_PP
  return check_launch("ifx_gemm_bf16(pp)");
}

}
```

Baseline: 22.03 frames/s.

## Add 224-token ping-pong GEMM tile to cut padding waste on M

```diff
diff --git a/include/inferix_hip.h b/include/inferix_hip.h
--- a/include/inferix_hip.h
+++ b/include/inferix_hip.h
@@ -107,6 +107,7 @@
                   const ifx_epilogue* epi, void* stream);
 
 int64_t ifx_gemm_workspace_bytes(int32_t M, int32_t N, int32_t K);
+int32_t ifx_gemm_pp_tile_tokens(int32_t M, int32_t N, int32_t K, int32_t epilogue, int32_t with_workspace);
 int ifx_gemm_bf16_ws(const ifx_bf16* x, int32_t ldx, const ifx_bf16* w, const ifx_bf16* bias, ifx_bf16* y, int32_t ldy,
                      int32_t M, int32_t N, int32_t K, const ifx_epilogue* epi, void* workspace, int64_t workspace_bytes,
                      void* stream);
diff --git a/inferix_amd/_hip.py b/inferix_amd/_hip.py
--- a/inferix_amd/_hip.py
+++ b/inferix_amd/_hip.py
@@ -128,6 +128,7 @@
     "ifx_attn_fwd_dedup": (C.c_int, [_vp, _vp, C.POINTER(KvView), _i32, _i32, _i32, _i32, _f32, _vp]),
     "ifx_attn_fwd_ranges": (C.c_int, [_vp, _i32, _vp, _i32, C.POINTER(KvView), _i32, _i32, _i32, C.POINTER(_i32), C.POINTER(_i32), _f32, _vp]),
     "ifx_gemm_workspace_bytes": (C.c_int64, [_i32, _i32, _i32]),
+    "ifx_gemm_pp_tile_tokens": (_i32, [_i32, _i32, _i32, _i32, _i32]),
     "ifx_gemm_bf16_ws": (C.c_int, [_vp, _i32, _vp, _vp, _vp, _i32, _i32, _i32, _i32, C.POINTER(Epilogue), _vp, C.c_int64, _vp]),
 }
 
diff --git a/inferix_amd/csrc/ifx_core.hip b/inferix_amd/csrc/ifx_core.hip
--- a/inferix_amd/csrc/ifx_core.hip
+++ b/inferix_amd/csrc/ifx_core.hip
@@ -82,7 +82,7 @@
   if (key && !strcmp(key, "gemm_small_split") && (value == 0 || value == 1)) { ifx::g_gemm_small_split = value; return IFX_OK; }
   if (key && !strcmp(key, "attn_variant") && value >= 0 && value <= 7) { ifx::g_attn_variant = value; return IFX_OK; }
   if (key && !strcmp(key, "conv_variant") && value >= 0 && value <= 1) { ifx::g_conv_variant = value; return IFX_OK; }
-  if (key && !strcmp(key, "gemm_pp_variant") && value >= 0 && value <= 1) { ifx::g_gemm_pp_variant = value; return IFX_OK; }
+  if (key && !strcmp(key, "gemm_pp_variant") && value >= 0 && value <= 3) { ifx::g_gemm_pp_variant = value; return IFX_OK; }
   if (key && !strcmp(key, "attn_debug_counters") && (value == 0 || value == 1)) {
     if (value == 1) {
       if (ifx::g_attn_dbg == nullptr && hipMalloc((void**)&ifx::g_attn_dbg, 64) != hipSuccess) {
diff --git a/inferix_amd/csrc/ifx_gemm.hip b/inferix_amd/csrc/ifx_gemm.hip
--- a/inferix_amd/csrc/ifx_gemm.hip
+++ b/inferix_amd/csrc/ifx_gemm.hip
@@ -124,6 +124,12 @@
   }
 }
 
+static constexpr float PP224_STEP_US = 1.45f, PP224_SPLIT_STEP_US = 1.53f;
+static bool pp224_candidate(int M) {
+  if (gemm_pp_variant() == 2) return false;
+  const long t7 = (M + 223) / 224, t4 = (M + 255) / 256;
+  return 100L * M >= 99L * t7 * 224 && 100L * M <= 97L * t4 * 256;
+}
 static int pick_pp(int M, int N, int K, int mode, bool have_ws) {
   if (N % 64 != 0 || K % 64 != 0) return 0;
   if (have_ws && gemm_pp_split(N, K) && ((M + 255) / 256) * ((N + 255) / 256) <= 1024 && !(gemm_small_split() && M < 2048)) {
@@ -135,7 +141,10 @@
       const char* e = getenv("IFX_PP_SPLIT_TJ3");
       allow3 = e ? atoi(e) : 1;
     }
-    return (allow3 && i3 <= 2048 && t3 < t4 && mode != IFX_EPI_GELU_TANH) ? 3 : 4;
+    const int best = (allow3 && i3 <= 2048 && t3 < t4 && mode != IFX_EPI_GELU_TANH) ? 3 : 4;
+    const int i7 = ((M + 223) / 224) * tn * 2;
+    const float t7 = ((i7 + 255) / 256) * (steps * PP224_SPLIT_STEP_US + 9.f);
+    return (pp224_candidate(M) && i7 <= 2048 && t7 < (best == 3 ? t3 : t4)) ? 7 : best;
   }
   if (M < 1024) return 0;
   static const float step_us[5] = {0.f, 0.f, 1.2f, 1.4f, 1.6f};
@@ -148,6 +157,11 @@
     const float t = rounds * ((K / 64) * step_us[tj] + tile_us);
     if (t < best_t) best_t = t, best = tj, best_tiles = tiles;
   }
+  if (pp224_candidate(M)) {
+    const int tiles = ((M + 223) / 224) * ((N + 255) / 256);
+    const float t = ((tiles + 255) / 256) * ((K / 64) * PP224_STEP_US + tile_us);
+    if (t < best_t) best_t = t, best = 7, best_tiles = tiles;
+  }
   if (M < 2048 && best_tiles < 160) return 0;
   return best;
 }
@@ -200,6 +214,12 @@
   if (!gemm_small_split() || M >= 2048 || N > 2048 || N % 64 != 0 || K < 4096 || K % 64 != 0 || (K / 64) % 4 != 0) return false;
   const int items = ((M + 127) / 128) * ((N + 255) / 256) * 4;
   return items > 128 && items <= 256;
+}
+
+static int pp_tile_option(int tj) { return tj == 4 && gemm_pp_variant() == 3 ? 7 : tj; }
+static int pp_tile_for(int variant, int M, int N, int K, int mode, bool ws_ok) {
+  const int tj = variant == 0 ? pick_pp(M, N, K, mode, ws_ok) : (variant == 22 || variant == 25 ? 4 : variant == 23 ? 3 : 2);
+  return pp_tile_option(tj);
 }
 
 static int gemm_bf16_impl(const ifx_bf16* x, int32_t ldx, const ifx_bf16* w, const ifx_bf16* bias, ifx_bf16* y,
@@ -225,7 +245,7 @@
   if (epi != nullptr && epi->y2 != nullptr) {
     IFX_REQUIRE(mode == IFX_EPI_BIAS && wide_ok && N % 64 == 0 && !((uintptr_t)bias & 7) && (variant == 0 || (variant >= 22 && variant <= 25)),
                 "ifx_gemm_bf16: the second destination (y2) needs the bias epilogue, N %% 64 == 0, 8-byte aligned bias and the ping-pong tiles");
-    int tj = variant == 0 ? pick_pp(M, N, K, mode, false) : (variant == 22 || variant == 25 ? 4 : variant == 23 ? 3 : 2);
+    int tj = pp_tile_for(variant, M, N, K, mode, false);
     if (tj == 0) tj = 2;
     ea.y2 = epi->y2, ea.ldy2 = epi->ldy2, ea.split_col = epi->split_col;
     return launch_gemm_pp(x, ldx, w, y, ldy, M, N, K, mode, ea, (hipStream_t)stream, tj, nullptr);
@@ -247,8 +267,8 @@
     return launch_gemm_lds_dma(12, x, ldx, w, y, ldy, M, N, K, mode, ea, (hipStream_t)stream);
   if (wide_ok && (variant == 0 || (variant >= 22 && variant <= 25))) {
     const bool ws_ok = workspace != nullptr && workspace_bytes >= (int64_t)gemm_pp_workspace_bytes(M, N, K) && variant != 25;
-    int tj = variant == 0 ? pick_pp(M, N, K, mode, ws_ok) : (variant == 22 || variant == 25 ? 4 : variant == 23 ? 3 : 2);
-    const bool fits = N % 64 == 0 && pp_epilogue_fits(mode, ea, 32 * tj);
+    const int tj = pp_tile_for(variant, M, N, K, mode, ws_ok);
+    const bool fits = N % 64 == 0 && pp_epilogue_fits(mode, ea, gemm_pp_group_rows(tj));
     if (tj && (fits || variant != 0))
       return launch_gemm_pp(x, ldx, w, y, ldy, M, N, K, mode, ea, (hipStream_t)stream, tj, ws_ok ? workspace : nullptr);
   }
@@ -290,6 +310,20 @@
   return 0;
 }
 
+extern "C" int32_t ifx_gemm_pp_tile_tokens(int32_t M, int32_t N, int32_t K, int32_t epilogue, int32_t with_workspace) {
+  if (M <= 0 || N <= 0 || K <= 0 || K % BK != 0 || N % 8 != 0) return 0;
+  const int v = gemm_variant();
+  const int mode = epilogue == IFX_EPI_GELU_ERF ? IFX_EPI_GELU_TANH : epilogue;
+  if (v == 26 || (v >= 27 && v <= 29)) return with_workspace && N % 64 == 0 ? 128 : 0;
+  if (v == 0 && small_split_takes_pp_ks4(M, N, K) && with_workspace) return 128;
+  if (v == 0 && small_split_takes_tile12(M, N, K)) return 0;
+  if (!(v == 0 || (v >= 22 && v <= 25))) return 0;
+  const bool ws_ok = with_workspace && v != 25;
+  const int tj = pp_tile_for(v, M, N, K, mode, ws_ok);
+  if (tj == 0 || (v == 0 && N % 64 != 0)) return 0;
+  return 2 * gemm_pp_group_rows(tj);
+}
+
 extern "C" int ifx_gemm_bf16_ws(const ifx_bf16* x, int32_t ldx, const ifx_bf16* w, const ifx_bf16* bias, ifx_bf16* y,
                                 int32_t ldy, int32_t M, int32_t N, int32_t K, const ifx_epilogue* epi, void* workspace,
                                 int64_t workspace_bytes, void* stream) {
diff --git a/inferix_amd/csrc/ifx_gemm_epilogue.h b/inferix_amd/csrc/ifx_gemm_epilogue.h
--- a/inferix_amd/csrc/ifx_gemm_epilogue.h
+++ b/inferix_amd/csrc/ifx_gemm_epilogue.h
@@ -125,5 +125,6 @@
 size_t gemm_pp_stream_k_workspace_bytes();
 bool gemm_pp_split(int N, int K);
 size_t gemm_pp_workspace_bytes(int M, int N, int K);
+int gemm_pp_group_rows(int tj);
 
 }
diff --git a/inferix_amd/csrc/ifx_gemm_pp.hip b/inferix_amd/csrc/ifx_gemm_pp.hip
--- a/inferix_amd/csrc/ifx_gemm_pp.hip
+++ b/inferix_amd/csrc/ifx_gemm_pp.hip
@@ -56,7 +56,7 @@
 };
 }
 
-template <int EPI, int TJ, int KS, int Q8 = 0, int LW = 0>
+template <int EPI, int TJ, int KS, int Q8 = 0, int LW = 0, int TH = 2 * TJ>
 __global__ __launch_bounds__(LW ? 768 : 512, LW ? 3 : 2) void gemm_pp_kernel(const unsigned short* __restrict__ x, int ldx,
                                                          const unsigned short* __restrict__ w, unsigned short* __restrict__ y,
                                                          int ldy, int M, int N, int K, int tiles_m, int total, int per_xcd,
@@ -66,7 +66,10 @@
   using namespace gpp;
   static_assert(!LW || (TJ == 2 && KS == 1 && Q8 == 0), "the loader-wave form is the unsplit bf16 128-token tile");
   dbg = IFX_PP_LAB ? dbg : (dbg & 32);
-  constexpr int BM = 64 * TJ;
+  static_assert(TH == 2 * TJ || (TH == 7 && TJ == 4 && Q8 == 0 && LW == 0 && (KS == 1 || KS == 2)),
+                "the 224-token tile is the bf16 eight-wave 256-token tile less one 16-token block per group");
+  constexpr int GR = 16 * TH;
+  constexpr int BM = 2 * GR;
   constexpr int GM = 4;
   constexpr bool RES = EPI == IFX_EPI_RESIDUAL || EPI == IFX_EPI_GATE_RES;
   extern __shared__ __attribute__((aligned(16))) unsigned char smem[];
@@ -179,7 +182,7 @@
                        : l31 * 128 + (((2 * ks + hi) ^ ((l31 >> 1) & 7)) << 4);
   const int w_frag_off = (w4 >> 1) * SLOT + (w4 & 1) * 8192 + W_LO;
   const int x_frag_off = grp == 0 ? X_UP : X_DN;
-  bf16x8 fx[4][TJ], fw[4][2], fx16[2 * TJ][2];
+  bf16x8 fx[4][TJ], fw[4][2], fx16[TH][2];
   int rg = 0;
   int rw = 0;
   const int w_off_lw = (w4 >> 1) * SLOT + (w4 & 1) * 8192, x_off_lw = grp == 0 ? 0 : LX_DN;
@@ -194,7 +197,7 @@
 #pragma unroll
         for (int c = 0; c < 4; ++c) fw[c][kk] = *reinterpret_cast<const bf16x8*>(wst + lane_ks[kk] + c * 2048);
 #pragma unroll
-        for (int t = 0; t < 2 * TJ; ++t) fx16[t][kk] = *reinterpret_cast<const bf16x8*>(xst + lane_ks[kk] + t * 2048);
+        for (int t = 0; t < TH; ++t) fx16[t][kk] = *reinterpret_cast<const bf16x8*>(xst + lane_ks[kk] + t * 2048);
       }
     } else {
 #pragma unroll
@@ -209,11 +212,14 @@
   };
 
   f32x16 acc[2][TJ];
-  f32x4 acc16[4][2 * TJ];
+  f32x4 acc16[4][TH];
   auto quad = [&](int i, int j, int g) __attribute__((always_inline)) {
-    if constexpr (MF16) return acc16[g][2 * j + i];
+    if constexpr (MF16) return acc16[g][2 * j + i < TH ? 2 * j + i : 0];
     else return f32x4{acc[i][j][4 * g], acc[i][j][4 * g + 1], acc[i][j][4 * g + 2], acc[i][j][4 * g + 3]};
   };
+  auto has_blk = [&](int i, int j) __attribute__((always_inline)) { return 2 * j + i < TH; };
+  auto has_rows = [&](int j, int p) __attribute__((always_inline)) { return j * 32 + p * 8 < GR; };
+  auto img_quad = [&](int i, int j, int g) __attribute__((always_inline)) { return TH == 2 * TJ ? (i * TJ + j) * 4 + g : (2 * j + i) * 4 + g; };
   auto mfma16 = [&](bool first) __attribute__((always_inline)) {
     const f32x4 z = {0.f, 0.f, 0.f, 0.f};
 #pragma unroll
@@ -221,7 +227,7 @@
 #pragma unroll
       for (int c = 0; c < 4; ++c)
 #pragma unroll
-        for (int t = 0; t < 2 * TJ; ++t)
+        for (int t = 0; t < TH; ++t)
           acc16[c][t] = __builtin_amdgcn_mfma_f32_16x16x32_bf16(fw[c][kk], fx16[t][kk], first && kk == 0 ? z : acc16[c][t], 0, 0, 0);
   };
   auto q8_mfma = [&](int kk, int i, int j, const f32x16 c) __attribute__((always_inline)) {
@@ -286,7 +292,7 @@
   auto part_slot = [&](int i) __attribute__((always_inline)) {
     return SK ? sk_p : item_tile(i) * (KSD - 1) + (item_split(i) > 0 ? item_split(i) - 1 : 0);
   };
-  auto part_soff = [&](int i) __attribute__((always_inline)) { return part_slot(i) * (BM * BN * 4) + wave * (TJ * 8192); };
+  auto part_soff = [&](int i) __attribute__((always_inline)) { return part_slot(i) * (BM * BN * 4) + wave * (TH * 4096); };
   auto flag_of = [&](int i) __attribute__((always_inline)) { return part_slot(i); };
   auto dump_partial = [&](int i) __attribute__((always_inline)) {
     int ln = __builtin_amdgcn_mbcnt_hi(~0u, __builtin_amdgcn_mbcnt_lo(~0u, 0u));
@@ -298,8 +304,9 @@
       for (int j = 0; j < TJ; ++j)
 #pragma unroll
         for (int q = 0; q < 4; ++q) {
+          if (!has_blk(ii, j)) continue;
           const f32x4 v = quad(ii, j, q);
-          __builtin_amdgcn_raw_buffer_store_b128(__builtin_bit_cast(u32x4, v), rs_ws, ln * 16 + ((ii * TJ + j) * 4 + q) * 1024, so, 16);
+          __builtin_amdgcn_raw_buffer_store_b128(__builtin_bit_cast(u32x4, v), rs_ws, ln * 16 + img_quad(ii, j, q) * 1024, so, 16);
         }
   };
   int flag_pending = 0;
@@ -336,7 +343,7 @@
     const int part_n = KS != 1 ? item_parts(i_tile) : 0;
     const int e_n0 = min(n_base + w4 * 64, N - 64);
     const bool n_ok = n_base + w4 * 64 < N;
-    const int e_m0 = m_base + grp * (32 * TJ);
+    const int e_m0 = m_base + grp * GR;
     const bool has_bias = ea.bias != nullptr;
     const unsigned short* const bias_p = has_bias ? ea.bias : y;
     const unsigned bias_mask = has_bias ? 0xffffffffu : 0u;
@@ -382,6 +389,7 @@
       if constexpr (RES) {
 #pragma unroll
         for (int p = 0; p < 4; ++p) {
+          if (!has_rows(j, p)) continue;
           const int m = min(e_m0 + j * 32 + p * 8 + rr, M - 1);
           e_res[j & 1][p] = *reinterpret_cast<const u32x4*>(ea.residual + (size_t)m * ea.ld_res + e_n0 + cc * 8);
         }
@@ -390,7 +398,7 @@
     if constexpr (RES) {
       fetch_res(0);
       if constexpr (EPI == IFX_EPI_GATE_RES) {
-        const int m_hi = min(e_m0 + 32 * TJ - 1, M - 1);
+        const int m_hi = min(e_m0 + GR - 1, M - 1);
         const int g_lo = min(e_m0, M - 1) / ea.rows_per_group, g_hi = m_hi / ea.rows_per_group;
         e_split = (g_lo + 1) * ea.rows_per_group;
         e_gate[0] = *reinterpret_cast<const u32x4*>(ea.mod + ((size_t)g_lo * ea.mod_slots + ea.gate_slot) * N + e_n0 + cc * 8);
@@ -428,6 +436,7 @@
       for (int i = 0; i < 2; ++i) {
 #pragma unroll
         for (int g = 0; g < 4; ++g) {
+          if (MF16 && !has_blk(i, j)) continue;
           const f32x4 aq = quad(i, j, g);
           float v[4] = {aq[0], aq[1], aq[2], aq[3]};
           if constexpr (Q8 == 2 && KS <= 1) {
@@ -438,7 +447,7 @@
             f32x4 pq[KSD - 1];
 #pragma unroll
             for (int q = 0; q < KSD - 1; ++q)
-              pq[q] = __builtin_bit_cast(f32x4, __builtin_amdgcn_raw_buffer_load_b128(rs_ws, ln * 16 + ((i * TJ + j) * 4 + g) * 1024,
+              pq[q] = __builtin_bit_cast(f32x4, __builtin_amdgcn_raw_buffer_load_b128(rs_ws, ln * 16 + img_quad(i, j, g) * 1024,
                                                                                       part_so + q * (BM * BN * 4), 16));
             if constexpr (Q8 == 2) {
               int vi[4];
@@ -463,7 +472,7 @@
           if constexpr (SK) {
             for (int q = 0; q < part_n; ++q) {
               const f32x4 pq = __builtin_bit_cast(f32x4, __builtin_amdgcn_raw_buffer_load_b128(
-                                                             rs_ws, ln * 16 + ((i * TJ + j) * 4 + g) * 1024, part_so + q * (BM * BN * 4), 16));
+                                                             rs_ws, ln * 16 + img_quad(i, j, g) * 1024, part_so + q * (BM * BN * 4), 16));
 #pragma unroll
               for (int e = 0; e < 4; ++e) v[e] += pq[e];
             }
@@ -501,6 +510,7 @@
       wait_lds();
 #pragma unroll
       for (int p = 0; p < 4; ++p) {
+        if (!has_rows(j, p)) continue;
         const int mrow = p * 8 + rr;
         const int m = e_m0 + j * 32 + mrow;
         const u16x8 vv = *reinterpret_cast<const u16x8*>(rd + p * 1024 + ((cc ^ (mrow & 7)) << 4));
@@ -643,7 +653,7 @@
     }
   } else {
     req_x(cb, X_UP, 0);
-    req_x(ca, X_DN, 32 * TJ);
+    req_x(ca, X_DN, GR);
     if (cb.g < G) req_x(cb, X_UP, 0);
     if (G > 1) wait_vm_if<2 * TJ, !LW>();
     else wait_vm_if<TJ, !LW>();
@@ -656,12 +666,12 @@
       const bool lower = ca.g < G, upper = cb.g < G;
       if (reads_first) {
         read_frags();
-        if (lower) req_x(ca, X_DN, 32 * TJ);
+        if (lower) req_x(ca, X_DN, GR);
         if (upper) req_x(cb, X_UP, 0);
         PP_STAMP();
         PP_STAMP();
       } else {
-        if (lower) req_x(ca, X_DN, 32 * TJ);
+        if (lower) req_x(ca, X_DN, GR);
         if (upper) req_x(cb, X_UP, 0);
         PP_STAMP();
         PP_STAMP();
@@ -768,10 +778,18 @@
 size_t gemm_pp_workspace_bytes(int M, int N, int K) {
   if (!gemm_pp_split(N, K)) return 0;
   const size_t tn = (size_t)(N + 255) / 256;
-  const size_t t4 = (size_t)((M + 255) / 256) * tn, t3 = (size_t)((M + 191) / 192) * tn;
+  const size_t t4 = (size_t)((M + 255) / 256) * tn, t3 = (size_t)((M + 191) / 192) * tn, t7 = (size_t)((M + 223) / 224) * tn;
   if (t4 > 1024) return 0;
-  const size_t b4 = t4 * 256 * 256 * 4, b3 = t3 <= 1024 ? t3 * 192 * 256 * 4 : 0;
-  return 4096 + (b4 > b3 ? b4 : b3);
+  const size_t b4 = t4 * 256 * 256 * 4, b3 = t3 <= 1024 ? t3 * 192 * 256 * 4 : 0, b7 = t7 <= 1024 ? t7 * 224 * 256 * 4 : 0;
+  return 4096 + max(b4, max(b3, b7));
+}
+
+int gemm_pp_group_rows(int tj) { return tj == 7 ? 112 : 32 * tj; }
+static bool pp_gate_groups_fit(int M, int gr, int rows_per_group) {
+  if (rows_per_group >= gr) return true;
+  for (int m0 = 0; m0 < M; m0 += gr)
+    if (min(m0 + gr - 1, M - 1) / rows_per_group - m0 / rows_per_group > 1) return false;
+  return true;
 }
 
 size_t gemm_pp_small_workspace_bytes(int M, int N, int ks) {
@@ -796,8 +814,15 @@
     set_error("ifx_gemm_bf16: the ping-pong tile needs N and K to be multiples of 64 (N = %d, K = %d)", N, K);
     return IFX_EINVAL;
   }
-  if (mode == IFX_EPI_GATE_RES && ea.rows_per_group < 32 * tj) {
-    set_error("ifx_gemm_bf16: the ping-pong tile needs gate groups of at least %d rows (rows_per_group = %d)", 32 * tj, ea.rows_per_group);
+  const bool t224 = tj == 7;
+  const int group_rows = gemm_pp_group_rows(tj);
+  if (t224) tj = 4;
+  if (t224 && (q8 || stream_k || force_ks > 1)) {
+    set_error("ifx_gemm_bf16: the 224-token ping-pong tile takes bf16 operands, unsplit or with K split in two");
+    return IFX_EINVAL;
+  }
+  if (mode == IFX_EPI_GATE_RES && !pp_gate_groups_fit(M, group_rows, ea.rows_per_group)) {
+    set_error("ifx_gemm_bf16: the ping-pong tile needs gate groups of at least %d rows (rows_per_group = %d)", group_rows, ea.rows_per_group);
     return IFX_EINVAL;
   }
   if (!pp_epilogue_fits(mode, ea, 0)) {
@@ -814,7 +839,7 @@
     n_cu = cu_of_dev[dev];
   }
   if (n_cu <= 0) n_cu = 256;
-  const int BM = 64 * tj;
+  const int BM = 2 * group_rows;
   const int tiles_m = (M + BM - 1) / BM, tiles_n = (N + BN - 1) / BN;
   int ks = stream_k ? 0 : ((tj == 4 || (tj == 3 && !q8)) && workspace != nullptr && gemm_pp_split(N, q8 ? K / 2 : K) &&
                            tiles_m * tiles_n <= 1024) ? 2 : 1;
@@ -855,21 +880,22 @@
     if (e) trace = (unsigned long long*)strtoull(e, nullptr, 0);
   }
 #endif
-#define IFX_LAUNCH_PP(E, T, S, Q, L)                                                                                                 \
+#define IFX_LAUNCH_PP(E, T, S, Q, L, H)                                                                                               \
   do {                                                                                                                               \
     static bool attr_set = false;                                                                                                    \
     if (!attr_set) {                                                                                                                 \
-      (void)hipFuncSetAttribute((const void*)gemm_pp_kernel<E, T, S, Q, L>, hipFuncAttributeMaxDynamicSharedMemorySize, (int)LDS_BYTES); \
+      (void)hipFuncSetAttribute((const void*)gemm_pp_kernel<E, T, S, Q, L, H>, hipFuncAttributeMaxDynamicSharedMemorySize, (int)LDS_BYTES); \
       attr_set = true;                                                                                                               \
     }                                                                                                                                \
-    hipLaunchKernelGGL((gemm_pp_kernel<E, T, S, Q, L>), grid, dim3(L ? 768 : 512), LDS_BYTES, s, x, ldx, w, y, ldy, M, N, K, tiles_m, \
+    hipLaunchKernelGGL((gemm_pp_kernel<E, T, S, Q, L, H>), grid, dim3(L ? 768 : 512), LDS_BYTES, s, x, ldx, w, y, ldy, M, N, K, tiles_m, \
                        total, per_xcd, wg_per_xcd, ea, trace, dbg_launch, ws_part, ws_flag, err_word, spin_ticks);                   \
   } while (0)
-#define IFX_SWITCH_PP_L(T, S, Q, L)                                                                             \
+#define IFX_SWITCH_PP_LH(T, S, Q, L, H)                                                                         \
   {                                                                                                             \
-    const int rc = dispatch_epilogue(mode, "ifx_gemm(pp)", [&](auto epi_c) { IFX_LAUNCH_PP(decltype(epi_c)::value, T, S, Q, L); }); \
+    const int rc = dispatch_epilogue(mode, "ifx_gemm(pp)", [&](auto epi_c) { IFX_LAUNCH_PP(decltype(epi_c)::value, T, S, Q, L, H); }); \
     if (rc != IFX_OK) return rc;                                                                                \
   }
+#define IFX_SWITCH_PP_L(T, S, Q, L) IFX_SWITCH_PP_LH(T, S, Q, L, 2 * (T))
 #define IFX_SWITCH_PP(T, S, Q) IFX_SWITCH_PP_L(T, S, Q, 0)
   if (q8 && ks == 2) {
     if (q8_int8) { IFX_SWITCH_PP(4, 2, 2) }
@@ -890,15 +916,18 @@
   } else if (tj == 2 && ks == 4) { IFX_SWITCH_PP(2, 4, 0)
   } else if (tj == 2 && ks == 8) { IFX_SWITCH_PP(2, 8, 0)
   } else if (ks == 2) {
-    if (tj == 4) { IFX_SWITCH_PP(4, 2, 0) }
+    if (t224) { IFX_SWITCH_PP_LH(4, 2, 0, 0, 7) }
+    else if (tj == 4) { IFX_SWITCH_PP(4, 2, 0) }
     else { IFX_SWITCH_PP(3, 2, 0) }
-  } else if (tj == 4) { IFX_SWITCH_PP(4, 1, 0) }
+  } else if (t224) { IFX_SWITCH_PP_LH(4, 1, 0, 0, 7) }
+  else if (tj == 4) { IFX_SWITCH_PP(4, 1, 0) }
   else if (tj == 3) { IFX_SWITCH_PP(3, 1, 0) }
   else if (tj == 2 && gemm_pp_variant() == 1) { IFX_SWITCH_PP(2, 1, 0) }
   else if (tj == 2) { IFX_SWITCH_PP_L(2, 1, 0, 1) }
   else { set_error("ifx_gemm_bf16: no ping-pong tile of %d tokens", 64 * tj); return IFX_EINVAL; }
 #undef IFX_SWITCH_PP
 #undef IFX_SWITCH_PP_L
+#undef IFX_SWITCH_PP_LH
 #undef IFX_LAUNCH_PP
   return check_launch("ifx_gemm_bf16(pp)");
 }
```

Result: no change. 21.90 frames/s (-0.6%).
